# uncbiag/DeepAtlas

Measured on AMD Instinct MI355X. Metric: training volumes/sec at 160x192x160 fp32; Dice vs CPU ref, higher is better.
Workload: dtype f32; 1 GPU; seg-only UNet_light + softmax-Dice + Adam training step, batch 2/GPU, 160x192x160 fp32 (BASELINE configs[1]); global_batch=2, n_classes=32, parallelism=dp1, matrix_precision=fp32_split, hip_graph=False, matrix_arithmetic_bits=22

## Files before the change

deepatlas_amd/_native.py:

```python
import ctypes
import os
from ctypes import c_int, c_float, c_longlong, c_size_t, c_void_p, c_char_p, POINTER

import torch

_HERE = os.path.dirname(os.path.abspath(__file__))
LIB_PATH = os.environ.get('DA_LIB') or os.path.join(_HERE, 'csrc', 'libdeepatlas_hip.so')

P = c_void_p
I = c_int
F = c_float
LL = c_longlong
SZ = c_size_t

SIGNATURES = {
    'da_version': (I, []),
    'da_device_info': (I, [POINTER(c_int), POINTER(c_int), POINTER(c_size_t), c_char_p, I]),
    'da_w_oik_to_tio': (I, [P, P, I, I, I, P]),
    'da_w_tio_to_oik': (I, [P, P, I, I, I, P]),
    'da_w_iok_to_tio': (I, [P, P, I, I, I, P]),
    'da_w_tio_to_iok': (I, [P, P, I, I, I, P]),
    'da_w_iok_flip_to_tio': (I, [P, P, I, I, I, P]),
    'da_w_tio_to_iok_flip': (I, [P, P, I, I, I, P]),
    'da_w_tio_to_oik_acc': (I, [P, P, I, I, I, P]),
    'da_w_tio_to_iok_acc': (I, [P, P, I, I, I, P]),
    'da_w_tio_to_iok_flip_acc': (I, [P, P, I, I, I, P]),
    'da_conv3d_k3_ws_bytes': (SZ, [I, I, I, I, I, I, I]),
    'da_conv3d_k3_pack_bytes': (SZ, [I, I, I, I, I, I]),
    'da_conv3d_k3_dgrad_bst': (I, [P, P, P, I, P, I, I, I, I, I, I, P, P, F, P, I, P, P, SZ, P]),
    'da_conv3d_k3_prepack': (I, [P, I, I, I, I, I, I, I, I, P, SZ, P, SZ, P, P]),
    'da_conv3d_k3_use_prepacked': (None, [P, P, SZ, P, SZ]),
    'da_conv3d_k3_prepack_many': (I, [I, P, P, P, P, P, P, P, P, P, P, P, P, P, P, P]),
    'da_conv3d_k3_fwd': (I, [P, I, P, I, P, P, P, I, I, I, I, I, I, F, P, SZ, P]),
    'da_conv3d_k3_fwd_bnstats': (I, [P, I, P, I, P, P, P, I, I, I, I, I, I, P, I, POINTER(c_int), P, SZ, P]),
    'da_conv3d_k3_dgrad': (I, [P, P, P, I, P, I, I, I, I, I, I, I, P, SZ, P]),
    'da_conv3d_k3_wgrad': (I, [P, I, P, I, P, P, P, I, I, I, I, I, I, P, SZ, P]),
    'da_conv3d_k3_fwd_pro': (I, [P, I, P, P, F, P, I, P, P, F, P, P, P, I, I, I, I, I, F, P, I, POINTER(c_int), P, SZ, P]),
    'da_conv3d_k3_wgrad_pro': (I, [P, I, P, P, F, P, I, P, P, F, P, P, I, I, I, I, I, P, SZ, P]),
    'da_upconv3d_k3_supported': (I, [I, I, I]),
    'da_upconv3d_k3_ws_bytes': (SZ, [I, I, I, I, I, I]),
    'da_upconv3d_k3_fwd': (I, [P, I, P, I, P, P, P, I, I, I, I, I, F, P, SZ, P]),
    'da_upconv3d_k3_dgrad': (I, [P, P, P, I, P, I, I, I, I, I, I, P, SZ, P]),
    'da_upconv3d_k3_wgrad': (I, [P, I, P, I, P, P, I, I, I, I, I, P, SZ, P]),
    'da_set_conv_direct': (I, [I]),
    'da_set_matrix_bf16': (I, [I]),
    'da_set_matrix_mode': (I, [I]),
    'da_pointwise_ws_bytes': (SZ, [I, I, I]),
    'da_conv1x1_fwd': (I, [P, P, P, P, LL, I, I, P, SZ, P]),
    'da_conv1x1_fwd_pro': (I, [P, P, P, F, P, P, P, LL, I, I, P, SZ, P]),
    'da_conv1x1_wgrad_pro': (I, [P, P, P, F, P, P, P, LL, I, I, P, SZ, P]),
    'da_conv1x1_dgrad': (I, [P, P, P, LL, I, I, P, SZ, P]),
    'da_conv1x1_wgrad_ws_bytes': (SZ, [LL, I, I]),
    'da_conv1x1_wgrad': (I, [P, P, P, P, LL, I, I, P, SZ, P]),
    'da_deconv_k2s2_fwd': (I, [P, P, P, P, I, I, I, I, I, I, P, SZ, P]),
    'da_deconv_k2s2_fwd_bnstats': (I, [P, P, P, P, I, I, I, I, I, I, P, I, POINTER(c_int), P, SZ, P]),
    'da_deconv_k2s2_dgrad': (I, [P, P, P, I, I, I, I, I, I, P, SZ, P]),
    'da_deconv_k2s2_bn_bwd_ws_bytes': (SZ, [I, I, I, I, I, I]),
    'da_deconv_k2s2_bn_bwd': (I, [P, P, P, P, P, P, F, P, P, P, P, P, P, P, I, I, I, I, I, I, P, I, P, SZ, P]),
    'da_deconv_k2s2_wgrad_ws_bytes': (SZ, [I, I, I, I, I, I]),
    'da_deconv_k2s2_wgrad': (I, [P, P, P, P, I, I, I, I, I, I, P, SZ, P]),
    'da_bn_ws_bytes': (SZ, [LL, I]),
    'da_bn_train_stats': (I, [P, LL, I, P, P, F, F, P, P, P, P, P, P, P, SZ, P]),
    'da_bn_train_stats_from_partials': (I, [P, I, LL, I, P, P, F, F, P, P, P, P, P, P, P]),
    'da_bn_eval_affine': (I, [P, P, P, P, F, I, P, P, P, P, P]),
    'da_bn_act_fwd': (I, [P, P, P, F, P, LL, I, P]),
    'da_bn_act_bwd': (I, [P, P, P, P, P, P, P, F, I, P, P, P, LL, I, P, SZ, P]),
    'da_bn_act_bwd_dbias': (I, [P, P, P, P, P, P, F, I, P, P, P, P, LL, I, P, SZ, P]),
    'da_bn_act_bwd_dbias_pre': (I, [P, P, P, P, P, P, F, I, P, P, P, P, LL, I, P, I, P, SZ, P]),
    'da_act_bwd': (I, [P, P, F, P, LL, P]),
    'da_act_bwd_add_dbias': (I, [P, P, P, F, P, P, LL, I, P, SZ, P]),
    'da_colsum': (I, [P, LL, I, P, P, SZ, P]),
    'da_act_bwd_add_partial': (I, [P, P, P, F, P, LL, I, P, SZ, POINTER(c_int), P]),
    'da_colsum_finish': (I, [P, I, I, P, I, P]),
    'da_maxpool2_fwd': (I, [P, P, I, I, I, I, I, P]),
    'da_maxpool2_fwd_pro': (I, [P, P, P, F, P, P, I, I, I, I, I, P]),
    'da_maxpool2_bwd': (I, [P, P, P, I, I, I, I, I, P]),
    'da_maxpool2_bwd_add': (I, [P, P, P, P, I, I, I, I, I, P]),
    'da_maxpool2_bwd_bst': (I, [P, P, P, P, I, I, I, I, I, P, F, P, I, P, P]),
    'da_upsample_nearest_fwd': (I, [P, P, I, I, I, I, I, I, I, I, P]),
    'da_upsample_nearest_bwd': (I, [P, P, I, I, I, I, I, I, I, I, P]),
    'da_warp_fwd': (I, [P, P, P, P, I, I, I, I, I, P]),
    'da_warp_bwd': (I, [P, P, P, P, P, I, I, I, I, I, P]),
    'da_label_warp_dice_ws_bytes': (SZ, [I, I]),
    'da_warp_dice_ws_bytes': (SZ, [I, I]),
    'da_warp_dice_fwd': (I, [P, P, P, I, I, I, I, I, I, I, I, F, P, P, P, SZ, P]),
    'da_softmax_dice_fwd': (I, [P, P, I, P, I, LL, I, I, I, F, P, P, P, SZ, P]),
    'da_label_warp_dice_fwd': (I, [P, I, P, I, P, I, I, I, I, I, I, I, F, P, P, P, SZ, P]),
    'da_label_warp_dice_bwd': (I, [P, I, P, I, P, P, P, P, I, I, I, I, I, P]),
    'da_softwarp_dice_ws_bytes': (SZ, [I, I]),
    'da_softwarp_dice_fwd': (I, [P, I, P, P, I, I, I, I, I, I, I, I, F, P, P, P, SZ, P]),
    'da_softwarp_dice_bwd_disp': (I, [P, I, P, P, P, P, P, I, I, I, I, I, P]),
    'da_softwarp_dice_bwd_logits': (I, [P, I, P, P, P, P, P, I, I, I, I, I, P]),
    'da_warp_adjoint_labels': (I, [P, I, P, P, P, I, I, I, I, I, P]),
    'da_seg_anat_dlogits': (I, [P, P, I, P, P, P, P, P, P, P, I, LL, I, P]),
    'da_warp_bwd_dsrc_det_ws_bytes': (SZ, [I, I, I, I, I]),
    'da_warp_bwd_dsrc_det': (I, [P, P, P, I, I, I, I, I, P, SZ, P]),
    'da_identity_grid': (I, [P, I, I, I, I, P]),
    'da_warp_labels_fwd': (I, [P, I, P, P, I, I, I, I, I, P]),
    'da_warp_labels_bwd': (I, [P, P, I, P, P, I, I, I, I, I, P]),
    'da_dice_ws_bytes': (SZ, [I, LL, I]),
    'da_dice_fwd': (I, [P, P, I, P, I, LL, I, I, I, I, F, P, P, P, SZ, P]),
    'da_dice_bwd': (I, [P, P, I, P, P, P, P, I, LL, I, I, P]),
    'da_softmax_fwd': (I, [P, P, LL, I, P]),
    'da_softmax_bwd': (I, [P, P, P, LL, I, P]),
    'da_one_hot': (I, [P, I, P, LL, I, P]),
    'da_head_dice_ws_bytes': (SZ, [I, LL, I, I]),
    'da_head_dice_fwd': (I, [P, P, P, F, P, P, P, I, I, LL, I, I, I, I, F, P, P, P, SZ, P]),
    'da_head_dice_bwd': (I, [P, P, P, F, P, P, P, I, P, P, P, P, P, I, LL, I, I, P, SZ, P]),
    'da_head_dice_bwd_bst': (I, [P, P, P, F, P, P, P, P, I, P, P, P, P, P, I, LL, I, I, P, I, P, P, SZ, P]),
    'da_ncc_ws_bytes': (SZ, [I, LL]),
    'da_ncc_fwd': (I, [P, P, I, LL, P, P, P, SZ, P]),
    'da_ncc_bwd': (I, [P, P, P, P, P, P, I, LL, P]),
    'da_bending_ws_bytes': (SZ, [I, I, I, I]),
    'da_bending_fwd': (I, [P, I, I, I, I, P, I, I, P, P, SZ, P]),
    'da_bending_bwd': (I, [P, P, P, I, I, I, I, P, I, I, P]),
    'da_xent_ws_bytes': (SZ, []),
    'da_xent_fwd': (I, [P, P, I, P, P, LL, I, I, I, F, LL, I, P, P, P, SZ, P]),
    'da_xent_bwd': (I, [P, P, I, P, P, P, P, P, LL, I, I, I, F, LL, P]),
    'da_argmax_dice_counts': (I, [P, P, I, I, LL, I, P, P, P]),
    'da_label_overlap_counts': (I, [P, I, P, I, I, LL, I, P, P]),
    'da_warp_labels_nearest_counts': (I, [P, I, P, I, P, I, I, I, I, I, P, P, P]),
    'da_jacobian_det_ws_bytes': (SZ, [I, I, I, I]),
    'da_jacobian_det': (I, [P, I, I, I, I, P, P, P, SZ, P]),
    'da_jacdet_penalty_ws_bytes': (SZ, [I, I, I, I]),
    'da_jacdet_penalty_fwd': (I, [P, I, I, I, I, F, I, P, P, P, P, SZ, P]),
    'da_jacdet_penalty_bwd': (I, [P, P, P, P, I, I, I, I, F, I, P]),
    'da_invcons_ws_bytes': (SZ, [I, I, I, I]),
    'da_invcons_fwd': (I, [P, P, I, I, I, I, P, P, P, P, SZ, P]),
    'da_invcons_bwd': (I, [P, P, P, P, P, P, I, I, I, I, I, P, SZ, P]),
    'da_field_invert_ws_bytes': (SZ, [I, I, I, I]),
    'da_field_invert': (I, [P, P, P, I, I, I, I, I, F, P, P, SZ, P]),
    'da_field_points_ws_bytes': (SZ, [I, I]),
    'da_field_transport_points': (I, [P, P, P, I, I, I, I, I, I, I, F, P, P, SZ, P]),
    'da_affine_warp_fwd': (I, [P, P, P, I, I, I, I, I, P]),
    'da_affine_warp_ws_bytes': (SZ, [I, I, I, I]),
    'da_affine_warp_bwd_theta': (I, [P, P, P, P, I, I, I, I, I, P, SZ, P]),
    'da_affine_compose_disp': (I, [P, P, P, I, I, I, I, P]),
    'da_label_fusion_vote': (I, [P, I, LL, P, P, P, I, I, I, I, I, P, P, P]),
    'da_local_msd_weights_ws_bytes': (SZ, [I, I, I, I, I]),
    'da_local_msd_weights': (I, [P, P, I, I, I, I, I, I, F, P, P, SZ, P]),
    'da_conv_k2s2_fwd': (I, [P, P, P, P, I, I, I, I, I, I, P, SZ, P]),
    'da_conv_k2s2_dgrad': (I, [P, P, P, I, I, I, I, I, I, P, SZ, P]),
    'da_conv_k2s2_wgrad_ws_bytes': (SZ, [I, I, I, I, I, I]),
    'da_conv_k2s2_wgrad': (I, [P, P, P, P, I, I, I, I, I, I, P, SZ, P]),
    'da_upsample_trilinear2_fwd': (I, [P, P, I, I, I, I, I, P]),
    'da_upsample_trilinear2_bwd': (I, [P, P, I, I, I, I, I, P]),
    'da_clamp01_to_f32': (I, [P, I, P, LL, P]),
    'da_crop3d': (I, [P, P, I, LL, I, I, I, I, I, I, I, I, I, P]),
    'da_partition_tiles': (I, [P, P, I, I, I, I, P, P, P]),
    'da_assemble_tiles': (I, [P, P, I, I, I, I, P, P, I, P]),
    'da_synth_volume': (I, [P, P, I, I, I, I, I, I, F, ctypes.c_uint, I, P]),
    'da_spatial_resample': (I, [P, P, I, I, P, P, I, P, P, I, I, I, I, I, I, I, I, P]),
    'da_lncc_ws_bytes': (SZ, [I, I, I, I, I, I, I]),
    'da_lncc_fwd': (I, [P, P, I, I, I, I, I, I, I, F, P, P, P, SZ, P]),
    'da_lncc_bwd': (I, [P, P, P, P, P, P, I, I, I, I, I, I, I, F, P, SZ, P]),
    'da_mi_ws_bytes': (SZ, [I, LL, I]),
    'da_mi_fwd': (I, [P, P, I, LL, I, F, F, F, P, P, P, SZ, P]),
    'da_mi_bwd': (I, [P, P, P, P, P, P, I, LL, I, F, F, F, P]),
    'da_gradloss_ws_bytes': (SZ, [I, I, I, I]),
    'da_gradloss_fwd': (I, [P, I, I, I, I, P, I, I, P, P, SZ, P]),
    'da_gradloss_bwd': (I, [P, P, P, I, I, I, I, P, I, I, P]),
    'da_adam_step': (I, [P, P, P, P, LL, F, F, F, F, I, F, P]),
    'da_adam_host_state': (I, [F, F, F, F, I, F, P]),
    'da_adam_step_dev': (I, [P, P, P, P, LL, P, P]),
}

BF16_TWINS = ['da_bn_train_stats', 'da_bn_act_fwd', 'da_bn_act_bwd_dbias', 'da_act_bwd', 'da_act_bwd_add_dbias', 'da_act_bwd_add_partial', 'da_colsum',
              'da_maxpool2_fwd', 'da_maxpool2_fwd_pro', 'da_maxpool2_bwd', 'da_maxpool2_bwd_add', 'da_upsample_nearest_fwd', 'da_upsample_nearest_bwd',
              'da_deconv_k2s2_fwd', 'da_deconv_k2s2_fwd_bnstats', 'da_deconv_k2s2_dgrad', 'da_deconv_k2s2_wgrad',
              'da_conv1x1_fwd', 'da_conv1x1_fwd_pro', 'da_conv1x1_dgrad', 'da_conv1x1_wgrad', 'da_conv1x1_wgrad_pro', 'da_head_dice_fwd', 'da_head_dice_bwd']
BF16_MASKED_TWINS = ['da_conv3d_k3_fwd', 'da_conv3d_k3_fwd_bnstats', 'da_conv3d_k3_fwd_pro', 'da_conv3d_k3_wgrad_pro', 'da_conv3d_k3_dgrad', 'da_conv3d_k3_wgrad']
for _n in BF16_TWINS:
    SIGNATURES[_n + '_bf16'] = (SIGNATURES[_n][0], list(SIGNATURES[_n][1]))
for _n in BF16_MASKED_TWINS:
    SIGNATURES[_n + '_bf16'] = (SIGNATURES[_n][0], list(SIGNATURES[_n][1]) + [ctypes.c_uint])
SIGNATURES['da_cast_f32_to_bf16'] = (I, [P, P, LL, P])
SIGNATURES['da_cast_bf16_to_f32'] = (I, [P, P, LL, P])

_lib = None


class NativeError(RuntimeError):
    pass


def lib():
    global _lib
    if _lib is None:
        if not os.path.isfile(LIB_PATH):
            raise NativeError(
                "deepatlas_amd: %s is missing. Build it with `python -c 'import __graft_entry__ as g; g.build()'` "
                "(hipcc --offload-arch=gfx950). There is no CPU/eager fallback for the hot path." % LIB_PATH)
        l = ctypes.CDLL(LIB_PATH)
        for name, (res, args) in SIGNATURES.items():
            fn = getattr(l, name)
            fn.restype = res
            fn.argtypes = args
        _lib = l
    return _lib


_ERR = {-1: 'DA_ERR_BADARG', -2: 'DA_ERR_WS_SMALL', -3: 'DA_ERR_UNSUPPORTED'}


class CallProfiler:

    def __init__(self, names=None):
        self.names = set(names) if names else None
        self.records = {}

    def wants(self, name):
        return self.names is None or name in self.names

    def summary(self):
        out = {}
        for key, evs in self.records.items():
            out[key] = (len(evs), sum(a.elapsed_time(b) for a, b in evs))
        return out


profiler = None
n_calls = 0


def call(name, *args):
    global n_calls
    n_calls += 1
    prof = profiler
    base = name[:-5] if name.endswith('_bf16') else name
    if prof is not None and prof.wants(base):
        a, b = torch.cuda.Event(enable_timing=True), torch.cuda.Event(enable_timing=True)
        a.record()
        rc = getattr(lib(), name)(*args)
        b.record()
        key = (base, tuple(x for x in args if isinstance(x, int)) + (('bf16',) if base != name else ()))
        prof.records.setdefault(key, []).append((a, b))
    else:
        rc = getattr(lib(), name)(*args)
    if rc != 0:
        raise NativeError('%s failed: %s' % (name, _ERR.get(rc, 'hipError_t %d' % rc)))


def call_supported(name, *args):
    try:
        call(name, *args)
        return True
    except NativeError as e:
        if 'DA_ERR_UNSUPPORTED' in str(e):
            return False
        raise


def ptr(t):
    if t is None:
        return None
    return c_void_p(t.data_ptr())


def stream():
    return c_void_p(torch.cuda.current_stream().cuda_stream)


def require_cuda(*tensors):
    for t in tensors:
        if t is not None and not t.is_cuda:
            raise NativeError("deepatlas_amd ops run only on the GPU (HIP kernels); got a CPU tensor. "
                              "The CPU restatement lives in oracle/ and is test infrastructure only.")


class _Workspace:

    def __init__(self):
        self.buf = {}
        self.capture_tag = None

    def get(self, nbytes, device):
        nbytes = int(nbytes) + 256
        key = (device.type, device.index if device.index is not None else torch.cuda.current_device(), torch.cuda.current_stream().cuda_stream)
        if self.capture_tag is not None and torch.cuda.is_current_stream_capturing():
            key = key + (self.capture_tag, len([k for k in self.buf if k[:3] == key and len(k) == 5 and k[3] == self.capture_tag]))
            for k, b in self.buf.items():
                if len(k) == 5 and k[:4] == key[:4] and b.numel() >= nbytes:
                    return c_void_p(b.data_ptr()), c_size_t(b.numel())
        b = self.buf.get(key)
        if b is None or b.numel() < nbytes:
            b = torch.empty(int(nbytes * 1.25) + 4096, dtype=torch.uint8, device=device)
            self.buf[key] = b
        return c_void_p(b.data_ptr()), c_size_t(b.numel())


    def release(self, tag):
        for k in [k for k in self.buf if len(k) == 5 and k[3] == tag]:
            del self.buf[k]


workspace = _Workspace()
```

deepatlas_amd/csrc/headdice.hip:

```cpp
#include "common.h"

typedef float f32x4 __attribute__((ext_vector_type(4)));

namespace {

constexpr int kHdBlocks = 1024;
constexpr int MT = 4;
constexpr float kLog2e = 1.44269504088896341f;

struct HdP {
    const float* x; const float* ps; const float* pt; float pslope;
    const float* wp_fwd; const float* wp_bwd; const float* bias;
    const void* labels; int label_bytes;
    long long V; int N, K, C;
    double* partial;
    const float* coef; const float* dloss;
    float* dx; float* wpartial;
    const float* pmean; double* bst;
};

__device__ __forceinline__ float hd_act01(float z, float s) { return fmaxf(z, z * s); }
__device__ __forceinline__ long long hd_label(const void* labels, int label_bytes, long long i) {
    return label_bytes == 1 ? (long long)((const unsigned char*)labels)[i] : ((const long long*)labels)[i];
}

__global__ void hd_pack_kernel(const float* __restrict__ w, float* __restrict__ wp, int K, int N, int transposed) {
    const int KC = K / 16, NT = N / 16;
    const int total = NT * KC * 256;
    for (int idx = blockIdx.x * blockDim.x + threadIdx.x; idx < total; idx += gridDim.x * blockDim.x) {
        const int m = idx & 3, lane = (idx >> 2) & 63;
        int rest = idx >> 8;
        const int c = rest % KC; const int n = rest / KC;
        const int k = 16 * c + 4 * (lane >> 4) + m, j = 16 * n + (lane & 15);
        wp[idx] = transposed ? w[(size_t)j * K + k] : w[(size_t)k * N + j];
    }
}

typedef float f2 __attribute__((ext_vector_type(2)));
__device__ __forceinline__ f2 hd_lo(f32x4 v) { return __builtin_shufflevector(v, v, 0, 1); }
__device__ __forceinline__ f2 hd_hi(f32x4 v) { return __builtin_shufflevector(v, v, 2, 3); }
__device__ __forceinline__ f2 hd_bc(float x) { return (f2){x, x}; }

template <int KC, typename T>
__device__ __forceinline__ void hd_load(const HdP& p, const T* __restrict__ xs, long long vbase, int i, int g, float4 (&a)[MT][KC]) {
#pragma unroll
    for (int t = 0; t < MT; ++t) {
        const long long vox = min(vbase + t * 16 + i, p.V - 1);
#pragma unroll
        for (int c = 0; c < KC; ++c) a[t][c] = da_ldq(xs, (vox * p.K + 16 * c + 4 * g) >> 2);
    }
}
__device__ __forceinline__ void hd_labels(const HdP& p, long long lbase, long long vbase, int i, int g, int (&rel)[MT]) {
#pragma unroll
    for (int t = 0; t < MT; ++t) rel[t] = (int)((const unsigned char*)p.labels)[(lbase + min(vbase + t * 16 + i, p.V - 1)) * p.label_bytes];
}
__device__ __forceinline__ int hd_rel(const HdP& p, int lab, long long vox, int g) { return (vox < p.V ? lab : -1000) - 4 * g; }
template <int NT>
__device__ __forceinline__ void hd_mask(int rel, f2 (&mk)[NT][2]) {
#pragma unroll
    for (int n = 0; n < NT; ++n) {
        mk[n][0] = (f2){rel == 16 * n ? 1.f : 0.f, rel == 16 * n + 1 ? 1.f : 0.f};
        mk[n][1] = (f2){rel == 16 * n + 2 ? 1.f : 0.f, rel == 16 * n + 3 ? 1.f : 0.f};
    }
}

template <int KC, int NT, typename T = float>
__device__ __forceinline__ void hd_probs(const HdP& p, long long vbase, int i, int g, const float4 (&psc)[KC], const float4 (&psf)[KC],
                                         const float4 (&wf)[NT][KC], const float (&bv)[NT][4], float4 (&a)[MT][KC], f32x4 (&acc)[MT][NT]) {
    if (p.ps) {
#pragma unroll
        for (int c = 0; c < KC; ++c) {
            const float4 sc = psc[c], sf = psf[c];
#pragma unroll
            for (int t = 0; t < MT; ++t) {
                a[t][c].x = hd_act01(a[t][c].x * sc.x + sf.x, p.pslope); a[t][c].y = hd_act01(a[t][c].y * sc.y + sf.y, p.pslope);
                a[t][c].z = hd_act01(a[t][c].z * sc.z + sf.z, p.pslope); a[t][c].w = hd_act01(a[t][c].w * sc.w + sf.w, p.pslope);
                if constexpr (DaEl<T>::bf) a[t][c] = da_unpack_bf16x4(da_pack_bf16x4(a[t][c]));
            }
        }
    }
#pragma unroll
    for (int t = 0; t < MT; ++t)
#pragma unroll
        for (int n = 0; n < NT; ++n) acc[t][n] = (f32x4){bv[n][0], bv[n][1], bv[n][2], bv[n][3]};
#pragma unroll
    for (int c = 0; c < KC; ++c) {
#pragma unroll
        for (int n = 0; n < NT; ++n)
#pragma unroll
            for (int t = 0; t < MT; ++t) acc[t][n] = __builtin_amdgcn_mfma_f32_16x16x4f32(wf[n][c].x, a[t][c].x, acc[t][n], 0, 0, 0);
#pragma unroll
        for (int n = 0; n < NT; ++n)
#pragma unroll
            for (int t = 0; t < MT; ++t) acc[t][n] = __builtin_amdgcn_mfma_f32_16x16x4f32(wf[n][c].y, a[t][c].y, acc[t][n], 0, 0, 0);
#pragma unroll
        for (int n = 0; n < NT; ++n)
#pragma unroll
            for (int t = 0; t < MT; ++t) acc[t][n] = __builtin_amdgcn_mfma_f32_16x16x4f32(wf[n][c].z, a[t][c].z, acc[t][n], 0, 0, 0);
#pragma unroll
        for (int n = 0; n < NT; ++n)
#pragma unroll
            for (int t = 0; t < MT; ++t) acc[t][n] = __builtin_amdgcn_mfma_f32_16x16x4f32(wf[n][c].w, a[t][c].w, acc[t][n], 0, 0, 0);
    }
#pragma unroll
    for (int t = 0; t < MT; ++t) {
        const bool valid = vbase + t * 16 + i < p.V;
        float m = acc[t][0][0];
#pragma unroll
        for (int n = 0; n < NT; ++n)
#pragma unroll
            for (int reg = 0; reg < 4; ++reg) m = fmaxf(m, acc[t][n][reg]);
        m = da_rows_max(m);
        f2 s2 = (f2){0.f, 0.f};
#pragma unroll
        for (int n = 0; n < NT; ++n) {
#pragma unroll
            for (int reg = 0; reg < 4; ++reg) acc[t][n][reg] = __builtin_amdgcn_exp2f(acc[t][n][reg] - m);
            s2 += hd_lo(acc[t][n]) + hd_hi(acc[t][n]);
        }
        const float s = da_rows_sum(s2.x + s2.y);
        const f2 inv = hd_bc(valid ? __builtin_amdgcn_rcpf(s) : 0.f);
#pragma unroll
        for (int n = 0; n < NT; ++n) {
            const f2 lo = hd_lo(acc[t][n]) * inv, hi = hd_hi(acc[t][n]) * inv;
            acc[t][n] = (f32x4){lo.x, lo.y, hi.x, hi.y};
        }
    }
}

template <int NT>
__device__ __forceinline__ void hd_bias(const HdP& p, int g, float (&bv)[NT][4]) {
#pragma unroll
    for (int n = 0; n < NT; ++n)
#pragma unroll
        for (int reg = 0; reg < 4; ++reg) bv[n][reg] = p.bias ? p.bias[16 * n + 4 * g + reg] * kLog2e : 0.f;
}
template <int KC, int NT>
__device__ __forceinline__ void hd_weights(const HdP& p, int lane, float4 (&wf)[NT][KC]) {
#pragma unroll
    for (int n = 0; n < NT; ++n)
#pragma unroll
        for (int c = 0; c < KC; ++c) {
            const float4 w = reinterpret_cast<const float4*>(p.wp_fwd)[(n * KC + c) * 64 + lane];
            wf[n][c] = make_float4(w.x * kLog2e, w.y * kLog2e, w.z * kLog2e, w.w * kLog2e);
        }
}
template <int KC>
__device__ __forceinline__ void hd_prologue(const HdP& p, int g, float4 (&psc)[KC], float4 (&psf)[KC]) {
#pragma unroll
    for (int c = 0; c < KC; ++c) {
        psc[c] = p.ps ? *reinterpret_cast<const float4*>(p.ps + 16 * c + 4 * g) : make_float4(1.f, 1.f, 1.f, 1.f);
        psf[c] = p.ps ? *reinterpret_cast<const float4*>(p.pt + 16 * c + 4 * g) : make_float4(0.f, 0.f, 0.f, 0.f);
    }
}

template <int KC, int NT, typename T = float>
__global__ void __launch_bounds__(256) head_dice_fwd_kernel(HdP p) {
    __shared__ double sred[4][3][NT * 16];
    const int lane = threadIdx.x & 63, wave = threadIdx.x >> 6;
    const int i = lane & 15, g = lane >> 4;
    const int n_s = blockIdx.y;
    const T* xs = reinterpret_cast<const T*>(p.x) + (long long)n_s * p.V * p.K;
    const long long lbase = (long long)n_s * p.V;
    float4 wf[NT][KC]; float bv[NT][4]; float4 psc[KC], psf[KC];
    hd_bias<NT>(p, g, bv);
    hd_weights<KC, NT>(p, lane, wf);
    hd_prologue<KC>(p, g, psc, psf);
    f2 sI[NT][2], sS[NT][2], sT[NT][2];
#pragma unroll
    for (int n = 0; n < NT; ++n)
#pragma unroll
        for (int h = 0; h < 2; ++h) sI[n][h] = sS[n][h] = sT[n][h] = (f2){0.f, 0.f};
    const long long nchunks = (p.V + 255) / 256;
    float4 an[MT][KC]; int reln[MT];
    if ((long long)blockIdx.x < nchunks) { hd_load<KC, T>(p, xs, (long long)blockIdx.x * 256 + wave * 64, i, g, an); hd_labels(p, lbase, (long long)blockIdx.x * 256 + wave * 64, i, g, reln); }
    for (long long cb = blockIdx.x; cb < nchunks; cb += gridDim.x) {
        const long long vbase = cb * 256 + wave * 64;
        float4 a[MT][KC]; f32x4 acc[MT][NT]; int rel[MT];
#pragma unroll
        for (int t = 0; t < MT; ++t) {
            rel[t] = hd_rel(p, reln[t], vbase + t * 16 + i, g);
#pragma unroll
            for (int c = 0; c < KC; ++c) a[t][c] = an[t][c];
        }
        { const long long vn = min(cb + (long long)gridDim.x, nchunks - 1) * 256 + wave * 64; hd_load<KC, T>(p, xs, vn, i, g, an); hd_labels(p, lbase, vn, i, g, reln); }
        hd_probs<KC, NT, T>(p, vbase, i, g, psc, psf, wf, bv, a, acc);
#pragma unroll
        for (int t = 0; t < MT; ++t) {
            f2 mk[NT][2];
            hd_mask<NT>(rel[t], mk);
#pragma unroll
            for (int n = 0; n < NT; ++n) {
                const f2 lo = hd_lo(acc[t][n]), hi = hd_hi(acc[t][n]);
                sS[n][0] += lo; sS[n][1] += hi;
                sI[n][0] += lo * mk[n][0]; sI[n][1] += hi * mk[n][1];
                sT[n][0] += mk[n][0]; sT[n][1] += mk[n][1];
            }
        }
    }
#pragma unroll
    for (int n = 0; n < NT; ++n)
#pragma unroll
        for (int reg = 0; reg < 4; ++reg) {
            double a0 = (double)sI[n][reg >> 1][reg & 1], a1 = (double)sS[n][reg >> 1][reg & 1], a2 = (double)sT[n][reg >> 1][reg & 1];
#pragma unroll
            for (int o = 1; o < 16; o <<= 1) { a0 += __shfl_xor(a0, o); a1 += __shfl_xor(a1, o); a2 += __shfl_xor(a2, o); }
            if (i == 0) { const int c = 16 * n + 4 * g + reg; sred[wave][0][c] = a0; sred[wave][1][c] = a1; sred[wave][2][c] = a2; }
        }
    __syncthreads();
    for (int idx = threadIdx.x; idx < 3 * p.C; idx += blockDim.x) {
        const int k = idx / p.C, c = idx % p.C;
        p.partial[(((size_t)n_s * gridDim.x + blockIdx.x) * 3 + k) * p.C + c] = (sred[0][k][c] + sred[1][k][c]) + (sred[2][k][c] + sred[3][k][c]);
    }
}

template <int KC, int NT, typename T = float>
__global__ void __launch_bounds__(256) head_dice_bwd_kernel(HdP p) {
    constexpr int K = KC * 16, C = NT * 16, LDX = K + 4, LDD = C + 4;
    extern __shared__ __attribute__((aligned(16))) float lds[];
    const int lane = threadIdx.x & 63, wave = threadIdx.x >> 6;
    const int i = lane & 15, g = lane >> 4;
    float* xl = lds + wave * (64 * LDX + 64 * LDD);
    float* dl = xl + 64 * LDX;
    float4 wf[NT][KC]; float bv[NT][4]; float4 psc[KC], psf[KC];
    hd_bias<NT>(p, g, bv);
    hd_weights<KC, NT>(p, lane, wf);
    hd_prologue<KC>(p, g, psc, psf);
    float wd[KC][NT][4];
#pragma unroll
    for (int c = 0; c < KC; ++c)
#pragma unroll
        for (int n = 0; n < NT; ++n)
#pragma unroll
            for (int reg = 0; reg < 4; ++reg) wd[c][n][reg] = p.wp_bwd[(size_t)(16 * c + i) * C + 16 * n + 4 * g + reg];
    const float gl = p.dloss[0];
    f32x4 wacc[KC][NT];
#pragma unroll
    for (int c = 0; c < KC; ++c)
#pragma unroll
        for (int n = 0; n < NT; ++n) wacc[c][n] = (f32x4){0.f, 0.f, 0.f, 0.f};
    f2 db[NT][2];
#pragma unroll
    for (int n = 0; n < NT; ++n) db[n][0] = db[n][1] = (f2){0.f, 0.f};
    const bool bst = KC == 1 && p.bst != nullptr;
    float4 bsc = make_float4(0.f, 0.f, 0.f, 0.f), bsf = bsc, bmu = bsc;
    float bs1[4] = {0.f, 0.f, 0.f, 0.f}, bs2[4] = {0.f, 0.f, 0.f, 0.f};
    if (bst) { bsc = *reinterpret_cast<const float4*>(p.ps + 4 * g); bsf = *reinterpret_cast<const float4*>(p.pt + 4 * g); bmu = *reinterpret_cast<const float4*>(p.pmean + 4 * g); }
    const long long chunks_per_sample = (p.V + 255) / 256, nchunks = chunks_per_sample * p.N;
    float4 an[MT][KC]; int reln[MT];
    auto fetch = [&](long long cb) {
        const int n_s = (int)(cb / chunks_per_sample);
        const long long vbase = (cb - (long long)n_s * chunks_per_sample) * 256 + wave * 64;
        hd_load<KC, T>(p, reinterpret_cast<const T*>(p.x) + (long long)n_s * p.V * p.K, vbase, i, g, an);
        hd_labels(p, (long long)n_s * p.V, vbase, i, g, reln);
    };
    if ((long long)blockIdx.x < nchunks) fetch(blockIdx.x);
    for (long long cb = blockIdx.x; cb < nchunks; cb += gridDim.x) {
        const int n_s = (int)(cb / chunks_per_sample);
        const long long vbase = (cb - (long long)n_s * chunks_per_sample) * 256 + wave * 64;
        const T* xs = reinterpret_cast<const T*>(p.x) + (long long)n_s * p.V * p.K;
        T* dxs = reinterpret_cast<T*>(p.dx) + (long long)n_s * p.V * p.K;
        const float* c0 = p.coef + (size_t)n_s * p.C;
        const float* c1 = p.coef + (size_t)(p.N + n_s) * p.C;
        float4 a[MT][KC]; f32x4 acc[MT][NT]; int rel[MT];
#pragma unroll
        for (int t = 0; t < MT; ++t) {
            rel[t] = hd_rel(p, reln[t], vbase + t * 16 + i, g);
#pragma unroll
            for (int c = 0; c < KC; ++c) a[t][c] = an[t][c];
        }
        fetch(min(cb + (long long)gridDim.x, nchunks - 1));
        hd_probs<KC, NT, T>(p, vbase, i, g, psc, psf, wf, bv, a, acc);
#pragma unroll
        for (int t = 0; t < MT; ++t)
#pragma unroll
            for (int c = 0; c < KC; ++c) *reinterpret_cast<float4*>(xl + (t * 16 + i) * LDX + 16 * c + 4 * g) = a[t][c];
        f2 k0[NT][2], k1[NT][2];
#pragma unroll
        for (int n = 0; n < NT; ++n)
#pragma unroll
            for (int h = 0; h < 2; ++h) {
                k0[n][h] = (f2){c0[16 * n + 4 * g + 2 * h], c0[16 * n + 4 * g + 2 * h + 1]};
                k1[n][h] = (f2){c1[16 * n + 4 * g + 2 * h], c1[16 * n + 4 * g + 2 * h + 1]};
            }
#pragma unroll
        for (int t = 0; t < MT; ++t) {
            f2 mk[NT][2], gg[NT][2], pr[NT][2], dot2 = (f2){0.f, 0.f};
            hd_mask<NT>(rel[t], mk);
#pragma unroll
            for (int n = 0; n < NT; ++n) {
                pr[n][0] = hd_lo(acc[t][n]); pr[n][1] = hd_hi(acc[t][n]);
#pragma unroll
                for (int h = 0; h < 2; ++h) { gg[n][h] = k0[n][h] * mk[n][h] + k1[n][h]; dot2 += gg[n][h] * pr[n][h]; }
            }
            const f2 dot = hd_bc(da_rows_sum(dot2.x + dot2.y)), gl2 = hd_bc(gl);
#pragma unroll
            for (int n = 0; n < NT; ++n) {
                const f2 d0 = (gl2 * pr[n][0]) * (gg[n][0] - dot), d1 = (gl2 * pr[n][1]) * (gg[n][1] - dot);
                db[n][0] += d0; db[n][1] += d1;
                acc[t][n] = (f32x4){d0.x, d0.y, d1.x, d1.y};
                *reinterpret_cast<float4*>(dl + (t * 16 + i) * LDD + 16 * n + 4 * g) = make_float4(d0.x, d0.y, d1.x, d1.y);
            }
        }
#pragma unroll
        for (int t = 0; t < MT; ++t) {
            f32x4 dacc[KC];
#pragma unroll
            for (int c = 0; c < KC; ++c) dacc[c] = (f32x4){0.f, 0.f, 0.f, 0.f};
#pragma unroll
            for (int n = 0; n < NT; ++n)
#pragma unroll
                for (int reg = 0; reg < 4; ++reg)
#pragma unroll
                    for (int c = 0; c < KC; ++c) dacc[c] = __builtin_amdgcn_mfma_f32_16x16x4f32(wd[c][n][reg], acc[t][n][reg], dacc[c], 0, 0, 0);
            const long long vox = vbase + t * 16 + i;
            if (vox < p.V) {
#pragma unroll
                for (int c = 0; c < KC; ++c)
                    da_stq_nt(dxs, (vox * p.K + 16 * c + 4 * g) >> 2, make_float4(dacc[c][0], dacc[c][1], dacc[c][2], dacc[c][3]));
                if (bst) {
                    const float4 xr = da_ldq(xs, (vox * p.K + 4 * g) >> 2);
                    const float xv[4] = {xr.x, xr.y, xr.z, xr.w}, scv[4] = {bsc.x, bsc.y, bsc.z, bsc.w}, sfv[4] = {bsf.x, bsf.y, bsf.z, bsf.w}, muv[4] = {bmu.x, bmu.y, bmu.z, bmu.w};
#pragma unroll
                    for (int j = 0; j < 4; ++j) {
                        const float dz = dacc[0][j] * da_act_grad(xv[j] * scv[j] + sfv[j], p.pslope >= 1.f ? -1.f : p.pslope);
                        bs1[j] += dz; bs2[j] += dz * (xv[j] - muv[j]);
                    }
                }
            }
        }
        __builtin_amdgcn_wave_barrier();
#pragma unroll 4
        for (int s = 0; s < 16; ++s) {
            float av[KC], bw[NT];
#pragma unroll
            for (int c = 0; c < KC; ++c) av[c] = xl[(4 * s + g) * LDX + 16 * c + i];
#pragma unroll
            for (int n = 0; n < NT; ++n) bw[n] = dl[(4 * s + g) * LDD + 16 * n + i];
#pragma unroll
            for (int c = 0; c < KC; ++c)
#pragma unroll
                for (int n = 0; n < NT; ++n) wacc[c][n] = __builtin_amdgcn_mfma_f32_16x16x4f32(av[c], bw[n], wacc[c][n], 0, 0, 0);
        }
        __builtin_amdgcn_wave_barrier();
    }
    __syncthreads();
    float* red = lds;
    for (int w = 0; w < 4; ++w) {
        if (wave == w) {
#pragma unroll
            for (int c = 0; c < KC; ++c)
#pragma unroll
                for (int n = 0; n < NT; ++n)
#pragma unroll
                    for (int reg = 0; reg < 4; ++reg) {
                        const int idx = (16 * c + 4 * g + reg) * C + 16 * n + i;
                        red[idx] = (w == 0 ? 0.f : red[idx]) + wacc[c][n][reg];
                    }
#pragma unroll
            for (int n = 0; n < NT; ++n)
#pragma unroll
                for (int reg = 0; reg < 4; ++reg) {
                    float d = db[n][reg >> 1][reg & 1];
#pragma unroll
                    for (int o = 1; o < 16; o <<= 1) d += __shfl_xor(d, o);
                    const int cidx = K * C + 16 * n + 4 * g + reg;
                    if (i == 0) red[cidx] = (w == 0 ? 0.f : red[cidx]) + d;
                }
        }
        __syncthreads();
    }
    float* part = p.wpartial + (size_t)blockIdx.x * (K * C + C);
    for (int idx = threadIdx.x; idx < K * C + C; idx += blockDim.x) part[idx] = red[idx];
    if (bst) {
        __syncthreads();
        double* dred = reinterpret_cast<double*>(lds);
#pragma unroll
        for (int j = 0; j < 4; ++j) {
            double a0 = (double)bs1[j], a1 = (double)bs2[j];
#pragma unroll
            for (int o = 1; o < 16; o <<= 1) { a0 += __shfl_xor(a0, o); a1 += __shfl_xor(a1, o); }
            if (i == 0) { dred[(wave * 2 + 0) * 16 + 4 * g + j] = a0; dred[(wave * 2 + 1) * 16 + 4 * g + j] = a1; }
        }
        __syncthreads();
        if (threadIdx.x < 32) {
            const int k = threadIdx.x >> 4, c = threadIdx.x & 15;
            p.bst[((size_t)blockIdx.x * 2 + k) * 16 + c] = (dred[(0 * 2 + k) * 16 + c] + dred[(1 * 2 + k) * 16 + c]) + (dred[(2 * 2 + k) * 16 + c] + dred[(3 * 2 + k) * 16 + c]);
        }
    }
}

static bool hd_shape_ok(int K, int C) { return (K == 16 || K == 64) && (C == 16 || C == 32); }

}

extern "C" size_t da_head_dice_ws_bytes(int N, long long V, int Cin, int C) {
    (void)V;
    const size_t pack = da_align((size_t)2 * Cin * C * sizeof(float));
    const size_t fwd = da_align((size_t)N * kHdBlocks * 3 * C * sizeof(double)) + da_align((size_t)3 * N * C * sizeof(float));
    const size_t bwd = da_align((size_t)kHdBlocks * (Cin * C + C) * sizeof(float)) + da_align((size_t)(Cin * C + C) * sizeof(float));
    return pack + (fwd > bwd ? fwd : bwd);
}

template <int KC, int NT, typename T>
static int hd_launch_fwd(const HdP& p, int nblocks, hipStream_t st) {
    hipLaunchKernelGGL((head_dice_fwd_kernel<KC, NT, T>), dim3(nblocks, p.N), dim3(256), 0, st, p);
    DA_LAUNCH_CHECK();
    return 0;
}
template <int KC, int NT, typename T>
static int hd_launch_bwd(const HdP& p, int nblocks, hipStream_t st) {
    const size_t shm = (size_t)4 * (64 * (KC * 16 + 4) + 64 * (NT * 16 + 4)) * sizeof(float);
    return da_launch_lds<head_dice_bwd_kernel<KC, NT, T>>(dim3(nblocks), dim3(256), shm, st, p);
}

template <typename T>
static int head_dice_fwd_t(const float* x, const float* pro_scale, const float* pro_shift, float pro_slope,
                           const float* w_io, const float* bias, const void* labels, int label_bytes,
                           int N, long long V, int Cin, int C, int weight_type, int no_bg, float eps,
                           float* loss, float* coef, void* ws, size_t ws_bytes, void* stream) {
    if (!x || !w_io || !labels || !loss || !coef || N <= 0 || N > 64 || V <= 0 || (label_bytes != 1 && label_bytes != 8) ||
        ((pro_scale == nullptr) != (pro_shift == nullptr))) return DA_ERR_BADARG;
    if (!hd_shape_ok(Cin, C) || (pro_scale && pro_slope >= 1.f)) return DA_ERR_UNSUPPORTED;
    if (ws_bytes < da_head_dice_ws_bytes(N, V, Cin, C)) return DA_ERR_WS_SMALL;
    hipStream_t st = da_stream(stream);
    float* wp = (float*)ws;
    hipLaunchKernelGGL(hd_pack_kernel, dim3(da_grid(Cin * C, 256, 64)), dim3(256), 0, st, w_io, wp, Cin, C, 0);
    DA_LAUNCH_CHECK();
    char* rest = (char*)ws + da_align((size_t)2 * Cin * C * sizeof(float));
    double* partial = (double*)rest;
    float* isc = (float*)(rest + da_align((size_t)N * kHdBlocks * 3 * C * sizeof(double)));
    int nblocks = (int)da_cdiv(V, 256 * 2); if (nblocks > kHdBlocks) nblocks = kHdBlocks; if (nblocks < 1) nblocks = 1;
    HdP p;
    p.x = x; p.ps = pro_scale; p.pt = pro_shift; p.pslope = pro_scale ? (pro_slope < 0.f ? 1.f : pro_slope) : 1.f;
    p.wp_fwd = wp; p.wp_bwd = nullptr; p.bias = bias; p.labels = labels; p.label_bytes = label_bytes;
    p.V = V; p.N = N; p.K = Cin; p.C = C; p.partial = partial; p.coef = nullptr; p.dloss = nullptr; p.dx = nullptr; p.wpartial = nullptr; p.pmean = nullptr; p.bst = nullptr;
    int rc;
    if (Cin == 16 && C == 32) rc = hd_launch_fwd<1, 2, T>(p, nblocks, st);
    else if (Cin == 16 && C == 16) rc = hd_launch_fwd<1, 1, T>(p, nblocks, st);
    else if (Cin == 64 && C == 32) rc = hd_launch_fwd<4, 2, T>(p, nblocks, st);
    else rc = hd_launch_fwd<4, 1, T>(p, nblocks, st);
    if (rc) return rc;
    return da_dice_finish(partial, nblocks, N, C, weight_type, no_bg, eps, loss, coef, isc, st);
}
extern "C" int da_head_dice_fwd(const float* x, const float* pro_scale, const float* pro_shift, float pro_slope,
                                const float* w_io, const float* bias, const void* labels, int label_bytes,
                                int N, long long V, int Cin, int C, int weight_type, int no_bg, float eps,
                                float* loss, float* coef, void* ws, size_t ws_bytes, void* stream) {
    return head_dice_fwd_t<float>(x, pro_scale, pro_shift, pro_slope, w_io, bias, labels, label_bytes, N, V, Cin, C, weight_type, no_bg, eps, loss, coef, ws, ws_bytes, stream);
}
extern "C" int da_head_dice_fwd_bf16(const void* x, const float* pro_scale, const float* pro_shift, float pro_slope,
                                     const float* w_io, const float* bias, const void* labels, int label_bytes,
                                     int N, long long V, int Cin, int C, int weight_type, int no_bg, float eps,
                                     float* loss, float* coef, void* ws, size_t ws_bytes, void* stream) {
    return head_dice_fwd_t<da_bf16>((const float*)x, pro_scale, pro_shift, pro_slope, w_io, bias, labels, label_bytes, N, V, Cin, C, weight_type, no_bg, eps, loss, coef, ws, ws_bytes, stream);
}

template <typename T>
static int head_dice_bwd_t(const float* x, const float* pro_scale, const float* pro_shift, float pro_slope,
                           const float* w_io, const float* bias, const void* labels, int label_bytes,
                           const float* coef, const float* dloss, float* dx, float* dw_io, float* dbias,
                           int N, long long V, int Cin, int C, void* ws, size_t ws_bytes, void* stream,
                           const float* pro_mean = nullptr, double* bst = nullptr, int bst_cap = 0, int* bst_n = nullptr) {
    if (bst_n) *bst_n = 0;
    if (!x || !w_io || !labels || !coef || !dloss || !dx || !dw_io || N <= 0 || V <= 0 || (label_bytes != 1 && label_bytes != 8) ||
        ((pro_scale == nullptr) != (pro_shift == nullptr))) return DA_ERR_BADARG;
    if (!hd_shape_ok(Cin, C) || (pro_scale && pro_slope >= 1.f)) return DA_ERR_UNSUPPORTED;
    if (ws_bytes < da_head_dice_ws_bytes(N, V, Cin, C)) return DA_ERR_WS_SMALL;
    hipStream_t st = da_stream(stream);
    float* wpf = (float*)ws;
    const float* wpb = w_io;
    hipLaunchKernelGGL(hd_pack_kernel, dim3(da_grid(Cin * C, 256, 64)), dim3(256), 0, st, w_io, wpf, Cin, C, 0);
    DA_LAUNCH_CHECK();
    char* rest = (char*)ws + da_align((size_t)2 * Cin * C * sizeof(float));
    float* wpartial = (float*)rest;
    const int O = Cin * C + C;
    float* folded = (float*)(rest + da_align((size_t)kHdBlocks * O * sizeof(float)));
    const long long nchunks = da_cdiv(V, 256) * N;
    int nblocks = (int)(nchunks < kHdBlocks ? nchunks : kHdBlocks); if (nblocks < 1) nblocks = 1;
    HdP p;
    p.x = x; p.ps = pro_scale; p.pt = pro_shift; p.pslope = pro_scale ? (pro_slope < 0.f ? 1.f : pro_slope) : 1.f;
    p.wp_fwd = wpf; p.wp_bwd = wpb; p.bias = bias; p.labels = labels; p.label_bytes = label_bytes;
    p.V = V; p.N = N; p.K = Cin; p.C = C; p.partial = nullptr; p.coef = coef; p.dloss = dloss; p.dx = dx; p.wpartial = wpartial;
    const bool want_bst = bst && pro_scale && pro_mean && Cin == 16 && bst_cap >= nblocks && !DaEl<T>::bf;
    p.pmean = want_bst ? pro_mean : nullptr; p.bst = want_bst ? bst : nullptr;
    if (want_bst && bst_n) *bst_n = nblocks;
    int rc;
    if (Cin == 16 && C == 32) rc = hd_launch_bwd<1, 2, T>(p, nblocks, st);
    else if (Cin == 16 && C == 16) rc = hd_launch_bwd<1, 1, T>(p, nblocks, st);
    else if (Cin == 64 && C == 32) rc = hd_launch_bwd<4, 2, T>(p, nblocks, st);
    else rc = hd_launch_bwd<4, 1, T>(p, nblocks, st);
    if (rc) return rc;
    rc = da_reduce_partials(wpartial, nblocks, O, folded, st);
    if (rc) return rc;
    hipError_t e = hipMemcpyAsync(dw_io, folded, (size_t)Cin * C * sizeof(float), hipMemcpyDeviceToDevice, st);
    if (e != hipSuccess) return (int)e;
    if (dbias) { e = hipMemcpyAsync(dbias, folded + (size_t)Cin * C, (size_t)C * sizeof(float), hipMemcpyDeviceToDevice, st); if (e != hipSuccess) return (int)e; }
    return 0;
}
extern "C" int da_head_dice_bwd(const float* x, const float* pro_scale, const float* pro_shift, float pro_slope,
                                const float* w_io, const float* bias, const void* labels, int label_bytes,
                                const float* coef, const float* dloss, float* dx, float* dw_io, float* dbias,
                                int N, long long V, int Cin, int C, void* ws, size_t ws_bytes, void* stream) {
    return head_dice_bwd_t<float>(x, pro_scale, pro_shift, pro_slope, w_io, bias, labels, label_bytes, coef, dloss, dx, dw_io, dbias, N, V, Cin, C, ws, ws_bytes, stream);
}
extern "C" int da_head_dice_bwd_bst(const float* x, const float* pro_scale, const float* pro_shift, float pro_slope, const float* pro_mean,
                                    const float* w_io, const float* bias, const void* labels, int label_bytes,
                                    const float* coef, const float* dloss, float* dx, float* dw_io, float* dbias,
                                    int N, long long V, int Cin, int C, double* bst, int bst_cap, int* bst_n, void* ws, size_t ws_bytes, void* stream) {
    return head_dice_bwd_t<float>(x, pro_scale, pro_shift, pro_slope, w_io, bias, labels, label_bytes, coef, dloss, dx, dw_io, dbias, N, V, Cin, C, ws, ws_bytes, stream,
                                  pro_mean, bst, bst_cap, bst_n);
}
extern "C" int da_head_dice_bwd_bf16(const void* x, const float* pro_scale, const float* pro_shift, float pro_slope,
                                     const float* w_io, const float* bias, const void* labels, int label_bytes,
                                     const float* coef, const float* dloss, void* dx, float* dw_io, float* dbias,
                                     int N, long long V, int Cin, int C, void* ws, size_t ws_bytes, void* stream) {
    return head_dice_bwd_t<da_bf16>((const float*)x, pro_scale, pro_shift, pro_slope, w_io, bias, labels, label_bytes, coef, dloss, (float*)dx, dw_io, dbias, N, V, Cin, C, ws, ws_bytes, stream);
}
```

deepatlas_amd/csrc/losses.hip:

```cpp
#include "common.h"

namespace {

constexpr int kBlocks = 512;
constexpr int kBendBlocks = 4096;
constexpr int kDiceBlocks = 2048;

__device__ __forceinline__ long long load_label(const void* labels, int label_bytes, long long i) {
    return label_bytes == 1 ? (long long)((const unsigned char*)labels)[i] : ((const long long*)labels)[i];
}

__device__ __forceinline__ void group_softmax4(float (&x)[4], int lpv) {
    float m = fmaxf(fmaxf(x[0], x[1]), fmaxf(x[2], x[3]));
    for (int o = 1; o < lpv; o <<= 1) m = fmaxf(m, __shfl_xor(m, o));
    float s = 0.f;
#pragma unroll
    for (int j = 0; j < 4; ++j) { x[j] = expf(x[j] - m); s += x[j]; }
    for (int o = 1; o < lpv; o <<= 1) s += __shfl_xor(s, o);
    const float inv = 1.f / s;
#pragma unroll
    for (int j = 0; j < 4; ++j) x[j] *= inv;
}

__global__ void dice_partial_vec_kernel(const float* __restrict__ src, const void* __restrict__ labels, int label_bytes,
                                        const float* __restrict__ soft, long long V, int C, int lpv, int softmax,
                                        double* __restrict__ partial, float* __restrict__ prob_out = nullptr) {
    extern __shared__ float shf[];
    const int n = blockIdx.y;
    const int slots = blockDim.x / lpv;
    const int q = threadIdx.x % lpv, s = threadIdx.x / lpv;
    float aI[4] = {0, 0, 0, 0}, aS[4] = {0, 0, 0, 0}, aT[4] = {0, 0, 0, 0};
    const long long vpb = da_cdiv(V, (long long)gridDim.x);
    const long long v0 = (long long)blockIdx.x * vpb;
    long long v1 = v0 + vpb; if (v1 > V) v1 = V;
    auto accumulate = [&](float4 a, const float* tt, long long row) {
        float p[4] = {a.x, a.y, a.z, a.w};
        if (softmax) group_softmax4(p, lpv);
        if (prob_out) *reinterpret_cast<float4*>(prob_out + row * C + q * 4) = make_float4(p[0], p[1], p[2], p[3]);
#pragma unroll
        for (int j = 0; j < 4; ++j) { aI[j] += p[j] * tt[j]; aS[j] += p[j]; aT[j] += tt[j]; }
    };
    auto target = [&](long long row, float* tt) {
        if (soft) {
            const float4 b = *reinterpret_cast<const float4*>(soft + row * C + q * 4);
            tt[0] = b.x; tt[1] = b.y; tt[2] = b.z; tt[3] = b.w;
        } else {
            const int lab = (int)load_label(labels, label_bytes, row) - q * 4;
#pragma unroll
            for (int j = 0; j < 4; ++j) tt[j] = (lab == j) ? 1.f : 0.f;
        }
    };
    long long v = v0 + s;
    for (; v + slots < v1; v += 2 * slots) {
        const long long r0 = (long long)n * V + v, r1 = r0 + slots;
        const float4 a0 = *reinterpret_cast<const float4*>(src + r0 * C + q * 4);
        const float4 a1 = *reinterpret_cast<const float4*>(src + r1 * C + q * 4);
        float t0[4], t1[4];
        target(r0, t0); target(r1, t1);
        accumulate(a0, t0, r0); accumulate(a1, t1, r1);
    }
    for (; v < v1; v += slots) {
        const long long r0 = (long long)n * V + v;
        const float4 a0 = *reinterpret_cast<const float4*>(src + r0 * C + q * 4);
        float t0[4];
        target(r0, t0);
        accumulate(a0, t0, r0);
    }
    float* sI = shf; float* sS = shf + (size_t)slots * C; float* sT = shf + (size_t)2 * slots * C;
#pragma unroll
    for (int j = 0; j < 4; ++j) { sI[s * C + q * 4 + j] = aI[j]; sS[s * C + q * 4 + j] = aS[j]; sT[s * C + q * 4 + j] = aT[j]; }
    __syncthreads();
    for (int c = threadIdx.x; c < C; c += blockDim.x) {
        double tI = 0, tS = 0, tT = 0;
        for (int k = 0; k < slots; ++k) { tI += sI[k * C + c]; tS += sS[k * C + c]; tT += sT[k * C + c]; }
        double* o = partial + (((size_t)n * gridDim.x + blockIdx.x) * 3) * C;
        o[c] = tI; o[C + c] = tS; o[2 * C + c] = tT;
    }
}

__global__ void dice_partial_gen_kernel(const float* __restrict__ src, const void* __restrict__ labels, int label_bytes,
                                        const float* __restrict__ soft, long long V, int C, int softmax,
                                        double* __restrict__ partial) {
    extern __shared__ float shf[];
    const int n = blockIdx.y;
    for (int c = threadIdx.x; c < 4 * 3 * C; c += blockDim.x) shf[c] = 0.f;
    __syncthreads();
    float* mine = shf + (threadIdx.x >> 6) * 3 * C;
    const long long vpb = da_cdiv(V, (long long)gridDim.x);
    const long long v0 = (long long)blockIdx.x * vpb;
    long long v1 = v0 + vpb; if (v1 > V) v1 = V;
    const long long span = da_cdiv(v1 - v0, (long long)blockDim.x) * blockDim.x;
    for (long long k = threadIdx.x; k < span; k += blockDim.x) {
        const long long v = v0 + k;
        const bool live = v < v1;
        const long long row = (long long)n * V + (live ? v : v0);
        float m = -INFINITY, ssum = 1.f;
        if (softmax) {
            for (int c = 0; c < C; ++c) m = fmaxf(m, src[row * C + c]);
            ssum = 0.f;
            for (int c = 0; c < C; ++c) ssum += expf(src[row * C + c] - m);
        }
        const int lab = soft ? -1 : (int)load_label(labels, label_bytes, row);
        for (int c = 0; c < C; ++c) {
            float p = src[row * C + c];
            if (softmax) p = expf(p - m) / ssum;
            float t = soft ? soft[row * C + c] : (lab == c ? 1.f : 0.f);
            if (!live) { p = 0.f; t = 0.f; }
            const float wI = da_wave_sum(p * t), wS = da_wave_sum(p), wT = da_wave_sum(t);
            if ((threadIdx.x & 63) == 0) { mine[c] += wI; mine[C + c] += wS; mine[2 * C + c] += wT; }
        }
    }
    __syncthreads();
    for (int c = threadIdx.x; c < C; c += blockDim.x) {
        double* o = partial + (((size_t)n * gridDim.x + blockIdx.x) * 3) * C;
        double a = 0.0, b = 0.0, t = 0.0;
        for (int w = 0; w < 4; ++w) { a += shf[w * 3 * C + c]; b += shf[w * 3 * C + C + c]; t += shf[w * 3 * C + 2 * C + c]; }
        o[c] = a; o[C + c] = b; o[2 * C + c] = t;
    }
}

__global__ void colreduce_inplace_kernel(double* __restrict__ partial, int N, int nblocks, int R) {
    const int wave = (int)((blockIdx.x * blockDim.x + threadIdx.x) >> 6), lane = threadIdx.x & 63;
    if (wave >= N * R) return;
    const int n = wave / R, r = wave % R;
    double* col = partial + (size_t)n * nblocks * R + r;
    double s = 0.0;
    for (int b = lane; b < nblocks; b += 64) s += col[(size_t)b * R];
    s = da_wave_sum(s);
    if (lane == 0) col[0] = s;
}

__global__ void dice_finalize_kernel(const double* __restrict__ partial, int nblocks, int nsum, int N, int C,
                                     int weight_type, int no_bg, float eps, float* __restrict__ loss,
                                     float* __restrict__ coef, float* __restrict__ isc ) {
    const int NC = N * C;
    for (int i = threadIdx.x; i < 3 * NC; i += blockDim.x) {
        const int k = i / NC, nc = i % NC, n = nc / C, c = nc % C;
        double s = 0.0;
        for (int b = 0; b < nsum; ++b) s += partial[(((size_t)n * nblocks + b) * 3 + k) * C + c];
        isc[i] = (float)s;
    }
    __syncthreads();
    if (threadIdx.x != 0) return;
    const float* I = isc; const float* S = isc + NC; const float* T = isc + 2 * NC;
    const int c0 = no_bg ? 1 : 0;
    float wmax = -INFINITY;
    for (int n = 0; n < N; ++n) {
        float rowmax = -INFINITY;
        for (int c = c0; c < C; ++c) {
            float w;
            if (weight_type == 1) w = 1.f / (powf(T[n * C + c], (float)(1.0 / 3.0)) + eps);
            else if (weight_type == 2) w = 1.f / (T[n * C + c] + eps);
            else w = 1.f;
            coef[n * C + c] = w;
            if (weight_type == 2) { const float t = isinf(w) ? 1.f : w; rowmax = fmaxf(rowmax, t); }
        }
        for (int c = c0; c < C; ++c) {
            float w = coef[n * C + c];
            if (weight_type == 2 && isinf(w)) { w = rowmax; coef[n * C + c] = w; }
            wmax = fmaxf(wmax, w);
        }
    }
    float wsum = 0.f, acc = 0.f;
    for (int n = 0; n < N; ++n)
        for (int c = c0; c < C; ++c) {
            const float w = coef[n * C + c] / wmax;
            coef[n * C + c] = w;
            const float score = (2.f * I[n * C + c] + eps) / ((S[n * C + c] + T[n * C + c]) + 2.f * eps);
            acc += w * score; wsum += w;
        }
    loss[0] = 1.f - acc / wsum;
    for (int n = 0; n < N; ++n)
        for (int c = 0; c < C; ++c) {
            if (c < c0) { coef[n * C + c] = 0.f; coef[NC + n * C + c] = 0.f; continue; }
            const float w = coef[n * C + c] / wsum;
            const float den = (S[n * C + c] + T[n * C + c]) + 2.f * eps;
            coef[n * C + c] = -w * 2.f / den;
            coef[NC + n * C + c] = w * (2.f * I[n * C + c] + eps) / (den * den);
        }
}

__global__ void dice_bwd_vec_kernel(const float* __restrict__ src, const void* __restrict__ labels, int label_bytes,
                                    const float* __restrict__ soft, const float* __restrict__ coef,
                                    const float* __restrict__ dloss, float* __restrict__ d_src,
                                    int N, long long V, int C, int lpv, int softmax) {
    const long long total = (long long)N * V * lpv;
    const float gl = dloss[0];
    const int NC = N * C;
    for (long long i = (long long)blockIdx.x * blockDim.x + threadIdx.x; i < total; i += (long long)gridDim.x * blockDim.x) {
        const int q = (int)(i % lpv);
        const long long row = i / lpv;
        const int n = (int)(row / V);
        const float4 a = *reinterpret_cast<const float4*>(src + row * C + q * 4);
        float p[4] = {a.x, a.y, a.z, a.w};
        if (softmax) group_softmax4(p, lpv);
        float t[4];
        if (soft) {
            const float4 b = *reinterpret_cast<const float4*>(soft + row * C + q * 4);
            t[0] = b.x; t[1] = b.y; t[2] = b.z; t[3] = b.w;
        } else {
            const int lab = (int)load_label(labels, label_bytes, row) - q * 4;
#pragma unroll
            for (int j = 0; j < 4; ++j) t[j] = (lab == j) ? 1.f : 0.f;
        }
        float g[4];
#pragma unroll
        for (int j = 0; j < 4; ++j) g[j] = coef[n * C + q * 4 + j] * t[j] + coef[NC + n * C + q * 4 + j];
        float4 o;
        if (softmax) {
            float dot = g[0] * p[0] + g[1] * p[1] + g[2] * p[2] + g[3] * p[3];
            for (int k = 1; k < lpv; k <<= 1) dot += __shfl_xor(dot, k);
            o = make_float4(gl * p[0] * (g[0] - dot), gl * p[1] * (g[1] - dot), gl * p[2] * (g[2] - dot), gl * p[3] * (g[3] - dot));
        } else {
            o = make_float4(gl * g[0], gl * g[1], gl * g[2], gl * g[3]);
        }
        *reinterpret_cast<float4*>(d_src + row * C + q * 4) = o;
    }
}

__global__ void dice_bwd_gen_kernel(const float* __restrict__ src, const void* __restrict__ labels, int label_bytes,
                                    const float* __restrict__ soft, const float* __restrict__ coef,
                                    const float* __restrict__ dloss, float* __restrict__ d_src,
                                    int N, long long V, int C, int softmax) {
    const long long total = (long long)N * V;
    const float gl = dloss[0];
    const int NC = N * C;
    for (long long row = (long long)blockIdx.x * blockDim.x + threadIdx.x; row < total; row += (long long)gridDim.x * blockDim.x) {
        const int n = (int)(row / V);
        const int lab = soft ? -1 : (int)load_label(labels, label_bytes, row);
        float m = -INFINITY, ssum = 1.f, dot = 0.f;
        if (softmax) {
            for (int c = 0; c < C; ++c) m = fmaxf(m, src[row * C + c]);
            ssum = 0.f;
            for (int c = 0; c < C; ++c) ssum += expf(src[row * C + c] - m);
            for (int c = 0; c < C; ++c) {
                const float p = expf(src[row * C + c] - m) / ssum;
                const float t = soft ? soft[row * C + c] : (lab == c ? 1.f : 0.f);
                dot += (coef[n * C + c] * t + coef[NC + n * C + c]) * p;
            }
        }
        for (int c = 0; c < C; ++c) {
            const float t = soft ? soft[row * C + c] : (lab == c ? 1.f : 0.f);
            const float g = coef[n * C + c] * t + coef[NC + n * C + c];
            if (softmax) { const float p = expf(src[row * C + c] - m) / ssum; d_src[row * C + c] = gl * p * (g - dot); }
            else d_src[row * C + c] = gl * g;
        }
    }
}

__global__ void softmax_fwd_kernel(const float* __restrict__ x, float* __restrict__ y, long long M, int C, int lpv) {
    if (lpv > 0) {
        const long long total = M * lpv;
        for (long long i = (long long)blockIdx.x * blockDim.x + threadIdx.x; i < total; i += (long long)gridDim.x * blockDim.x) {
            const int q = (int)(i % lpv); const long long row = i / lpv;
            const float4 a = *reinterpret_cast<const float4*>(x + row * C + q * 4);
            float p[4] = {a.x, a.y, a.z, a.w};
            group_softmax4(p, lpv);
            *reinterpret_cast<float4*>(y + row * C + q * 4) = make_float4(p[0], p[1], p[2], p[3]);
        }
    } else {
        for (long long row = (long long)blockIdx.x * blockDim.x + threadIdx.x; row < M; row += (long long)gridDim.x * blockDim.x) {
            float m = -INFINITY, s = 0.f;
            for (int c = 0; c < C; ++c) m = fmaxf(m, x[row * C + c]);
            for (int c = 0; c < C; ++c) s += expf(x[row * C + c] - m);
            for (int c = 0; c < C; ++c) y[row * C + c] = expf(x[row * C + c] - m) / s;
        }
    }
}

__global__ void softmax_bwd_kernel(const float* __restrict__ dy, const float* __restrict__ y, float* __restrict__ dx,
                                   long long M, int C, int lpv) {
    if (lpv > 0) {
        const long long total = M * lpv;
        for (long long i = (long long)blockIdx.x * blockDim.x + threadIdx.x; i < total; i += (long long)gridDim.x * blockDim.x) {
            const int q = (int)(i % lpv); const long long row = i / lpv;
            const float4 g = *reinterpret_cast<const float4*>(dy + row * C + q * 4);
            const float4 p = *reinterpret_cast<const float4*>(y + row * C + q * 4);
            float dot = g.x * p.x + g.y * p.y + g.z * p.z + g.w * p.w;
            for (int k = 1; k < lpv; k <<= 1) dot += __shfl_xor(dot, k);
            *reinterpret_cast<float4*>(dx + row * C + q * 4) = make_float4(p.x * (g.x - dot), p.y * (g.y - dot), p.z * (g.z - dot), p.w * (g.w - dot));
        }
    } else {
        for (long long row = (long long)blockIdx.x * blockDim.x + threadIdx.x; row < M; row += (long long)gridDim.x * blockDim.x) {
            float dot = 0.f;
            for (int c = 0; c < C; ++c) dot += dy[row * C + c] * y[row * C + c];
            for (int c = 0; c < C; ++c) dx[row * C + c] = y[row * C + c] * (dy[row * C + c] - dot);
        }
    }
}

__global__ void one_hot_kernel(const void* __restrict__ labels, int label_bytes, float* __restrict__ out, long long M, int C) {
    const long long total = M * C;
    for (long long i = (long long)blockIdx.x * blockDim.x + threadIdx.x; i < total; i += (long long)gridDim.x * blockDim.x) {
        const long long row = i / C; const int c = (int)(i % C);
        out[i] = ((int)load_label(labels, label_bytes, row) == c) ? 1.f : 0.f;
    }
}

static int lpv_for(int C) {
    if (C % 4 != 0) return 0;
    const int q = C / 4;
    if (q > 64 || (q & (q - 1)) != 0) return 0;
    return q;
}

template <bool ALIGNED>
__global__ void ncc_partial_kernel(const float* __restrict__ x, const float* __restrict__ y, long long V,
                                   double* __restrict__ partial ) {
    __shared__ double red[5][4];
    const int n = blockIdx.y;
    const float* xs = x + (long long)n * V; const float* ys = y + (long long)n * V;
    const float px = xs[0], py = ys[0];
    float a[5] = {0, 0, 0, 0, 0};
    double acc[5] = {0, 0, 0, 0, 0};
    long long head = 0;
    if (!ALIGNED) {
        head = (long long)(((16 - ((size_t)xs & 15)) & 15) >> 2);
        if ((((size_t)xs ^ (size_t)ys) & 15) != 0 || head > V) head = V;
    }
    const long long V4 = (V - head) / 4;
    const float* xb = xs + head; const float* yb = ys + head;
    int cnt = 0;
    for (long long i = (long long)blockIdx.x * blockDim.x + threadIdx.x; i < V4; i += (long long)gridDim.x * blockDim.x) {
        float4 p = reinterpret_cast<const float4*>(xb)[i];
        float4 q = reinterpret_cast<const float4*>(yb)[i];
        p.x -= px; p.y -= px; p.z -= px; p.w -= px;
        q.x -= py; q.y -= py; q.z -= py; q.w -= py;
        a[0] += (p.x + p.y) + (p.z + p.w);
        a[1] += (q.x + q.y) + (q.z + q.w);
        a[2] += (p.x * q.x + p.y * q.y) + (p.z * q.z + p.w * q.w);
        a[3] += (p.x * p.x + p.y * p.y) + (p.z * p.z + p.w * p.w);
        a[4] += (q.x * q.x + q.y * q.y) + (q.z * q.z + q.w * q.w);
        if (++cnt == 16) {
#pragma unroll
            for (int k = 0; k < 5; ++k) { acc[k] += (double)a[k]; a[k] = 0.f; }
            cnt = 0;
        }
    }
    if (ALIGNED) {
        if (blockIdx.x == 0) for (long long i = V4 * 4 + threadIdx.x; i < V; i += blockDim.x) {
            const float p = xs[i] - px, q = ys[i] - py;
            a[0] += p; a[1] += q; a[2] += p * q; a[3] += p * p; a[4] += q * q;
        }
    } else {
        const long long nscalar = V - V4 * 4;
        cnt = 0;
        for (long long j = (long long)blockIdx.x * blockDim.x + threadIdx.x; j < nscalar; j += (long long)gridDim.x * blockDim.x) {
            const long long i = j < head ? j : j + V4 * 4;
            const float p = xs[i] - px, q = ys[i] - py;
            a[0] += p; a[1] += q; a[2] += p * q; a[3] += p * p; a[4] += q * q;
            if (++cnt == 64) {
#pragma unroll
                for (int k = 0; k < 5; ++k) { acc[k] += (double)a[k]; a[k] = 0.f; }
                cnt = 0;
            }
        }
    }
#pragma unroll
    for (int k = 0; k < 5; ++k) acc[k] += (double)a[k];
    const int lane = threadIdx.x & 63, wid = threadIdx.x >> 6;
#pragma unroll
    for (int k = 0; k < 5; ++k) { const double w = da_wave_sum(acc[k]); if (lane == 0) red[k][wid] = w; }
    __syncthreads();
    if (threadIdx.x < 5) {
        double s = 0.0;
        for (int w = 0; w < (int)(blockDim.x >> 6); ++w) s += red[threadIdx.x][w];
        partial[((size_t)n * gridDim.x + blockIdx.x) * 5 + threadIdx.x] = s;
    }
}

__global__ void ncc_finalize_kernel(const double* __restrict__ partial, int nblocks, int nsum, int N, long long V,
                                    const float* __restrict__ x, const float* __restrict__ y,
                                    float* __restrict__ loss, double* __restrict__ stats) {
    __shared__ double sncc[64];
    const int n = threadIdx.x;
    if (n < N) {
        double s[5] = {0, 0, 0, 0, 0};
        for (int b = 0; b < nsum; ++b)
            for (int k = 0; k < 5; ++k) s[k] += partial[((size_t)n * nblocks + b) * 5 + k];
        const double M = (double)V;
        const double mx = s[0] / M, my = s[1] / M;
        const double cov = s[2] / M - mx * my;
        double vx = s[3] / M - mx * mx, vy = s[4] / M - my * my;
        const double ncc = cov / (sqrt(vx) * sqrt(vy));
        double* o = stats + (size_t)n * 8;
        o[0] = mx + (double)x[(long long)n * V]; o[1] = my + (double)y[(long long)n * V]; o[2] = cov; o[3] = vx; o[4] = vy; o[5] = ncc; o[6] = M; o[7] = 0.0;
        sncc[n] = ncc;
    }
    __syncthreads();
    if (threadIdx.x == 0) {
        double t = 0.0;
        for (int i = 0; i < N; ++i) t += sncc[i];
        loss[0] = (float)(1.0 - t / (double)N);
    }
}

__global__ void ncc_bwd_kernel(const float* __restrict__ x, const float* __restrict__ y, const double* __restrict__ stats,
                               const float* __restrict__ dloss, float* __restrict__ dx, float* __restrict__ dy,
                               int N, long long V) {
    const int n = blockIdx.y;
    const double* s = stats + (size_t)n * 8;
    const float mx = (float)s[0], my = (float)s[1];
    const double sxy = sqrt(s[3]) * sqrt(s[4]);
    const double k = -(double)dloss[0] / ((double)N * s[6]);
    const float ax = (float)(k / sxy), bx = (float)(-k * s[5] / s[3]);
    const float ay = (float)(k / sxy), by = (float)(-k * s[5] / s[4]);
    const float* xs = x + (long long)n * V; const float* ys = y + (long long)n * V;
    for (long long i = (long long)blockIdx.x * blockDim.x + threadIdx.x; i < V; i += (long long)gridDim.x * blockDim.x) {
        const float xt = xs[i] - mx, yt = ys[i] - my;
        if (dx) dx[(long long)n * V + i] = ax * yt + bx * xt;
        if (dy) dy[(long long)n * V + i] = ay * xt + by * yt;
    }
}

struct BendK { float k[3][6]; };

static BendK bending_coeffs(int N, int D, int H, int W, const float* spacing3, int normalize, int norm) {
    float sp[3] = {1.f, 1.f, 1.f};
    if (spacing3) { sp[0] = spacing3[0]; sp[1] = spacing3[1]; sp[2] = spacing3[2]; }
    if (normalize) { const float m = fminf(sp[0], fminf(sp[1], sp[2])); sp[0] /= m; sp[1] /= m; sp[2] /= m; }
    float dims[3] = {(float)D, (float)H, (float)W};
    if (normalize) { const float m = fminf(dims[0], fminf(dims[1], dims[2])); dims[0] /= m; dims[1] /= m; dims[2] /= m; }
    const float den[6] = {sp[0] * sp[0], sp[1] * sp[1], sp[2] * sp[2], sp[0] * sp[1], sp[1] * sp[2], sp[2] * sp[0]};
    const double Mint = (double)(D - 2) * (H - 2) * (W - 2);
    BendK K;
    for (int c = 0; c < 3; ++c)
        for (int t = 0; t < 6; ++t) {
            const float w = norm == 2 ? dims[c] * sp[c] / den[t] : 1.f;
            const double mult = (t < 3 ? 1.0 : 2.0) / (9.0 * 3.0 * (double)N * Mint);
            K.k[c][t] = (float)((double)(w * w) * mult);
        }
    return K;
}

#define BU(dd, hh, ww) u[((((long long)(dd)) * H + (hh)) * W + (ww)) * 3 + c]

struct F3 { float x, y, z; };
__device__ __forceinline__ F3 ld3(const float* __restrict__ u, long long vox) {
    const float* p = u + vox * 3;
    return F3{p[0], p[1], p[2]};
}

template <bool L1>
__global__ void bending_partial_kernel(const float* __restrict__ disp, int D, int H, int W, BendK K,
                                       double* __restrict__ partial) {
    __shared__ double red[4];
    const int n = blockIdx.y;
    const float* u = disp + (long long)n * D * H * W * 3;
    const int Di = D - 2, Hi = H - 2, Wi = W - 2;
    const long long total = (long long)Di * Hi * Wi;
    const long long sH = W, sD = (long long)H * W;
    float acc = 0.f; double dacc = 0.0; int cnt = 0;
    for (DaXcdLoop L = da_xcd_loop(total); L.i < L.end; L.i += L.step) {
        const long long i = L.i;
        long long r = i;
        const int w = (int)(r % Wi) + 1; r /= Wi;
        const int h = (int)(r % Hi) + 1; const int d = (int)(r / Hi) + 1;
        const long long p = ((long long)d * H + h) * W + w;
        const F3 c0 = ld3(u, p);
        const F3 dp = ld3(u, p + sD), dm = ld3(u, p - sD), hp = ld3(u, p + sH), hm = ld3(u, p - sH), wp = ld3(u, p + 1), wm = ld3(u, p - 1);
        const F3 dhpp = ld3(u, p + sD + sH), dhmm = ld3(u, p - sD - sH), dhpm = ld3(u, p + sD - sH), dhmp = ld3(u, p - sD + sH);
        const F3 hwpp = ld3(u, p + sH + 1), hwmm = ld3(u, p - sH - 1), hwpm = ld3(u, p + sH - 1), hwmp = ld3(u, p - sH + 1);
        const F3 dwpp = ld3(u, p + sD + 1), dwmm = ld3(u, p - sD - 1), dwpm = ld3(u, p + sD - 1), dwmp = ld3(u, p - sD + 1);
#define BEND_CH(f, c)                                                                                   \
        {                                                                                               \
            const float t0 = dp.f + dm.f - 2.f * c0.f, t1 = hp.f + hm.f - 2.f * c0.f, t2 = wp.f + wm.f - 2.f * c0.f;   \
            const float t3 = dhpp.f + dhmm.f - dhpm.f - dhmp.f;                                         \
            const float t4 = hwpp.f + hwmm.f - hwpm.f - hwmp.f;                                         \
            const float t5 = dwpp.f + dwmm.f - dwpm.f - dwmp.f;                                         \
            if (L1) acc += K.k[c][0] * fabsf(t0) + K.k[c][1] * fabsf(t1) + K.k[c][2] * fabsf(t2) + K.k[c][3] * fabsf(t3) + K.k[c][4] * fabsf(t4) + K.k[c][5] * fabsf(t5); \
            else acc += K.k[c][0] * t0 * t0 + K.k[c][1] * t1 * t1 + K.k[c][2] * t2 * t2 + K.k[c][3] * t3 * t3 + K.k[c][4] * t4 * t4 + K.k[c][5] * t5 * t5; \
        }
        BEND_CH(x, 0) BEND_CH(y, 1) BEND_CH(z, 2)
#undef BEND_CH
        if (++cnt == 16) { dacc += (double)acc; acc = 0.f; cnt = 0; }
    }
    dacc += (double)acc;
    const double s = da_block_sum(dacc, red);
    if (threadIdx.x == 0) partial[(size_t)n * gridDim.x + blockIdx.x] = s;
}

__global__ void scalar_finalize_kernel(const double* __restrict__ partial, int count, float* __restrict__ loss) {
    __shared__ double red[4];
    double s = 0.0;
    for (int i = threadIdx.x; i < count; i += blockDim.x) s += partial[i];
    s = da_block_sum(s, red);
    if (threadIdx.x == 0) loss[0] = (float)s;
}

template <bool L1>
__device__ __forceinline__ float bend_grad_elem(const float* __restrict__ u, int d, int h, int w, int c, int D, int H, int W, const BendK& K) {
    auto interior = [&](int dd, int hh, int ww) { return dd >= 1 && dd < D - 1 && hh >= 1 && hh < H - 1 && ww >= 1 && ww < W - 1; };
    auto f = [](float t) { return L1 ? (t > 0.f ? 1.f : (t < 0.f ? -1.f : 0.f)) : t; };
    float g = 0.f;
    {
        float s0 = 0.f, s1 = 0.f, s2 = 0.f;
        if (interior(d, h, w)) {
            const float u0 = BU(d, h, w);
            s0 -= 2.f * f(BU(d + 1, h, w) + BU(d - 1, h, w) - 2.f * u0);
            s1 -= 2.f * f(BU(d, h + 1, w) + BU(d, h - 1, w) - 2.f * u0);
            s2 -= 2.f * f(BU(d, h, w + 1) + BU(d, h, w - 1) - 2.f * u0);
        }
#pragma unroll
        for (int sgn = -1; sgn <= 1; sgn += 2) {
            if (interior(d + sgn, h, w)) s0 += f(BU(d + 2 * sgn, h, w) + BU(d, h, w) - 2.f * BU(d + sgn, h, w));
            if (interior(d, h + sgn, w)) s1 += f(BU(d, h + 2 * sgn, w) + BU(d, h, w) - 2.f * BU(d, h + sgn, w));
            if (interior(d, h, w + sgn)) s2 += f(BU(d, h, w + 2 * sgn) + BU(d, h, w) - 2.f * BU(d, h, w + sgn));
        }
        g += K.k[c][0] * s0 + K.k[c][1] * s1 + K.k[c][2] * s2;
    }
    {
        float s3 = 0.f, s4 = 0.f, s5 = 0.f;
#pragma unroll
        for (int sa = -1; sa <= 1; sa += 2)
#pragma unroll
            for (int sb = -1; sb <= 1; sb += 2) {
                const float cf = (float)(sa * sb);
                { const int qd = d - sa, qh = h - sb;
                  if (interior(qd, qh, w)) s3 += cf * f(BU(qd + 1, qh + 1, w) + BU(qd - 1, qh - 1, w) - BU(qd + 1, qh - 1, w) - BU(qd - 1, qh + 1, w)); }
                { const int qh = h - sa, qw = w - sb;
                  if (interior(d, qh, qw)) s4 += cf * f(BU(d, qh + 1, qw + 1) + BU(d, qh - 1, qw - 1) - BU(d, qh + 1, qw - 1) - BU(d, qh - 1, qw + 1)); }
                { const int qd = d - sa, qw = w - sb;
                  if (interior(qd, h, qw)) s5 += cf * f(BU(qd + 1, h, qw + 1) + BU(qd - 1, h, qw - 1) - BU(qd + 1, h, qw - 1) - BU(qd - 1, h, qw + 1)); }
            }
        g += K.k[c][3] * s3 + K.k[c][4] * s4 + K.k[c][5] * s5;
    }
    return g;
}

template <bool L1>
__global__ void bending_bwd_kernel(const float* __restrict__ disp, const float* __restrict__ dloss,
                                   float* __restrict__ d_disp, int D, int H, int W, BendK K) {
    const int n = blockIdx.y;
    const float* u = disp + (long long)n * D * H * W * 3;
    float* du = d_disp + (long long)n * D * H * W * 3;
    const long long total = (long long)D * H * W * 3;
    const float gl = (L1 ? 1.f : 2.f) * dloss[0];
    const long long sW = 3, sH = (long long)W * 3, sD = (long long)H * W * 3;
    for (DaXcdLoop L = da_xcd_loop(total, 768); L.i < L.end; L.i += L.step) {
        const long long i = L.i;
        const int c = (int)(i % 3); long long r = i / 3;
        const int w = (int)(r % W); r /= W;
        const int h = (int)(r % H); const int d = (int)(r / H);
        float g;
        const bool deep = !L1 && d >= 2 && d < D - 2 && h >= 2 && h < H - 2 && w >= 2 && w < W - 2;
        if (deep) {
            const float* q = u + i;
            const float c0 = q[0];
            const float d2 = q[2 * sD] + q[-2 * sD], d1 = q[sD] + q[-sD];
            const float h2 = q[2 * sH] + q[-2 * sH], h1 = q[sH] + q[-sH];
            const float w2 = q[2 * sW] + q[-2 * sW], w1 = q[sW] + q[-sW];
            const float dh = q[2 * sD + 2 * sH] + q[2 * sD - 2 * sH] + q[-2 * sD + 2 * sH] + q[-2 * sD - 2 * sH];
            const float hw = q[2 * sH + 2 * sW] + q[2 * sH - 2 * sW] + q[-2 * sH + 2 * sW] + q[-2 * sH - 2 * sW];
            const float dw = q[2 * sD + 2 * sW] + q[2 * sD - 2 * sW] + q[-2 * sD + 2 * sW] + q[-2 * sD - 2 * sW];
            g = K.k[c][0] * (d2 - 4.f * d1 + 6.f * c0) + K.k[c][1] * (h2 - 4.f * h1 + 6.f * c0) + K.k[c][2] * (w2 - 4.f * w1 + 6.f * c0) +
                K.k[c][3] * (4.f * c0 - 2.f * (d2 + h2) + dh) + K.k[c][4] * (4.f * c0 - 2.f * (h2 + w2) + hw) + K.k[c][5] * (4.f * c0 - 2.f * (d2 + w2) + dw);
        } else {
            g = bend_grad_elem<L1>(u, d, h, w, c, D, H, W, K);
        }
        du[i] = gl * g;
    }
}
#undef BU

__global__ void argmax_counts_kernel(const float* __restrict__ logits, const void* __restrict__ truth, int label_bytes,
                                     long long V, int C, int lpv, unsigned long long* __restrict__ counts,
                                     unsigned char* __restrict__ pred) {
    extern __shared__ unsigned int shc[];
    const int n = blockIdx.y;
    for (int c = threadIdx.x; c < 3 * C; c += blockDim.x) shc[c] = 0u;
    __syncthreads();
    const int L = lpv > 0 ? lpv : 1;
    const long long total = V * L;
    for (long long i = (long long)blockIdx.x * blockDim.x + threadIdx.x; i < total; i += (long long)gridDim.x * blockDim.x) {
        const int q = (int)(i % L); const long long v = i / L;
        const long long row = (long long)n * V + v;
        float best; int bi;
        if (lpv > 0) {
            const float4 a = *reinterpret_cast<const float4*>(logits + row * C + q * 4);
            best = a.x; bi = q * 4;
            if (a.y > best) { best = a.y; bi = q * 4 + 1; }
            if (a.z > best) { best = a.z; bi = q * 4 + 2; }
            if (a.w > best) { best = a.w; bi = q * 4 + 3; }
            for (int o = 1; o < lpv; o <<= 1) {
                const float ob = __shfl_xor(best, o); const int oi = __shfl_xor(bi, o);
                if (ob > best || (ob == best && oi < bi)) { best = ob; bi = oi; }
            }
        } else {
            best = logits[row * C]; bi = 0;
            for (int c = 1; c < C; ++c) { const float a = logits[row * C + c]; if (a > best) { best = a; bi = c; } }
        }
        if (q == 0) {
            const int t = (int)load_label(truth, label_bytes, row);
            atomicAdd(&shc[bi], 1u);
            if (t >= 0 && t < C) atomicAdd(&shc[C + t], 1u);
            if (t == bi) atomicAdd(&shc[2 * C + bi], 1u);
            if (pred) pred[row] = (unsigned char)bi;
        }
    }
    __syncthreads();
    for (int c = threadIdx.x; c < 3 * C; c += blockDim.x) {
        const int k = c / C, cc = c % C;
        if (shc[c]) atomicAdd(&counts[((size_t)n * C + cc) * 3 + k], (unsigned long long)shc[c]);
    }
}


__global__ void label_overlap_counts_kernel(const void* __restrict__ pred, int pred_bytes, const void* __restrict__ truth, int truth_bytes,
                                            long long V, int C, unsigned long long* __restrict__ counts) {
    extern __shared__ unsigned int shc[];
    constexpr int RUN = 16;
    const int n = blockIdx.y;
    for (int c = threadIdx.x; c < 4 * 3 * C; c += blockDim.x) shc[c] = 0u;
    __syncthreads();
    unsigned int* h = shc + (threadIdx.x >> 6) * 3 * C;
    auto flush = [&](int pl, int tl, unsigned int len) {
        if (len == 0u) return;
        if (pl >= 0 && pl < C) atomicAdd(&h[pl], len);
        if (tl >= 0 && tl < C) atomicAdd(&h[C + tl], len);
        if (pl == tl && pl >= 0 && pl < C) atomicAdd(&h[2 * C + pl], len);
    };
    const long long nruns = (V + RUN - 1) / RUN;
    for (long long r = (long long)blockIdx.x * blockDim.x + threadIdx.x; r < nruns; r += (long long)gridDim.x * blockDim.x) {
        const long long v0 = r * RUN;
        const int cnt = (int)((V - v0) < RUN ? (V - v0) : RUN);
        int pl = -1, tl = -1; unsigned int len = 0u;
        for (int k = 0; k < cnt; ++k) {
            const long long row = (long long)n * V + v0 + k;
            const int a = (int)load_label(pred, pred_bytes, row), b = (int)load_label(truth, truth_bytes, row);
            if (a != pl || b != tl) { flush(pl, tl, len); pl = a; tl = b; len = 0u; }
            ++len;
        }
        flush(pl, tl, len);
    }
    __syncthreads();
    for (int c = threadIdx.x; c < 3 * C; c += blockDim.x) {
        const unsigned int t = shc[c] + shc[3 * C + c] + shc[6 * C + c] + shc[9 * C + c];
        const int k = c / C, cc = c % C;
        if (t) atomicAdd(&counts[((size_t)n * C + cc) * 3 + k], (unsigned long long)t);
    }
}

}

extern "C" size_t da_dice_ws_bytes(int N, long long V, int C) {
    (void)V;
    return da_align((size_t)N * kDiceBlocks * 3 * C * sizeof(double)) + da_align((size_t)3 * N * C * sizeof(float));
}

extern "C" int da_dice_fwd(const float* src, const void* labels, int label_bytes, const float* soft_target,
                           int N, long long V, int C, int softmax, int weight_type, int no_bg, float eps,
                           float* loss, float* coef, void* ws, size_t ws_bytes, void* stream) {
    if (!src || (!labels && !soft_target) || !loss || !coef || N <= 0 || N > 64 || V <= 0 || C <= 0 || C > 256) return DA_ERR_BADARG;
    if (labels && label_bytes != 1 && label_bytes != 8) return DA_ERR_BADARG;
    if (ws_bytes < da_dice_ws_bytes(N, V, C)) return DA_ERR_WS_SMALL;
    hipStream_t st = da_stream(stream);
    double* partial = (double*)ws;
    float* isc = (float*)((char*)ws + da_align((size_t)N * kDiceBlocks * 3 * C * sizeof(double)));
    const int lpv = lpv_for(C);
    int nblocks = (int)da_cdiv(V, 256); if (nblocks > kDiceBlocks) nblocks = kDiceBlocks;
    if (lpv > 0) {
        const int slots = 256 / lpv;
        hipLaunchKernelGGL(dice_partial_vec_kernel, dim3(nblocks, N), dim3(256), (size_t)3 * slots * C * sizeof(float), st,
                           src, labels, label_bytes, soft_target, V, C, lpv, softmax, partial);
    } else {
        hipLaunchKernelGGL(dice_partial_gen_kernel, dim3(nblocks, N), dim3(256), (size_t)4 * 3 * C * sizeof(float), st,
                           src, labels, label_bytes, soft_target, V, C, softmax, partial);
    }
    DA_LAUNCH_CHECK();
    hipLaunchKernelGGL(colreduce_inplace_kernel, dim3((unsigned)da_cdiv((long long)N * 3 * C * 64, 256)), dim3(256), 0, st, partial, N, nblocks, 3 * C);
    DA_LAUNCH_CHECK();
    hipLaunchKernelGGL(dice_finalize_kernel, dim3(1), dim3(256), 0, st, partial, nblocks, 1, N, C, weight_type, no_bg, eps, loss, coef, isc);
    DA_LAUNCH_CHECK();
    return 0;
}

extern "C" int da_softmax_dice_fwd(const float* src, const void* labels, int label_bytes, float* prob,
                                   int N, long long V, int C, int weight_type, int no_bg, float eps,
                                   float* loss, float* coef, void* ws, size_t ws_bytes, void* stream) {
    if (!src || !labels || !prob || !loss || !coef || N <= 0 || N > 64 || V <= 0 || C <= 0 || C > 256) return DA_ERR_BADARG;
    if (label_bytes != 1 && label_bytes != 8) return DA_ERR_BADARG;
    const int lpv = lpv_for(C);
    if (lpv <= 0) return DA_ERR_UNSUPPORTED;
    if (ws_bytes < da_dice_ws_bytes(N, V, C)) return DA_ERR_WS_SMALL;
    hipStream_t st = da_stream(stream);
    double* partial = (double*)ws;
    float* isc = (float*)((char*)ws + da_align((size_t)N * kDiceBlocks * 3 * C * sizeof(double)));
    int nblocks = (int)da_cdiv(V, 256); if (nblocks > kDiceBlocks) nblocks = kDiceBlocks;
    const int slots = 256 / lpv;
    hipLaunchKernelGGL(dice_partial_vec_kernel, dim3(nblocks, N), dim3(256), (size_t)3 * slots * C * sizeof(float), st,
                       src, labels, label_bytes, (const float*)nullptr, V, C, lpv, 1, partial, prob);
    DA_LAUNCH_CHECK();
    return da_dice_finish(partial, nblocks, N, C, weight_type, no_bg, eps, loss, coef, isc, st);
}

int da_dice_finish(double* partial, int nblocks, int N, int C, int weight_type, int no_bg, float eps,
                   float* loss, float* coef, float* isc, hipStream_t st) {
    hipLaunchKernelGGL(colreduce_inplace_kernel, dim3((unsigned)da_cdiv((long long)N * 3 * C * 64, 256)), dim3(256), 0, st, partial, N, nblocks, 3 * C);
    DA_LAUNCH_CHECK();
    hipLaunchKernelGGL(dice_finalize_kernel, dim3(1), dim3(256), 0, st, partial, nblocks, 1, N, C, weight_type, no_bg, eps, loss, coef, isc);
    DA_LAUNCH_CHECK();
    return 0;
}

extern "C" int da_dice_bwd(const float* src, const void* labels, int label_bytes, const float* soft_target,
                           const float* coef, const float* dloss, float* d_src,
                           int N, long long V, int C, int softmax, void* stream) {
    if (!src || (!labels && !soft_target) || !coef || !dloss || !d_src || N <= 0 || V <= 0 || C <= 0) return DA_ERR_BADARG;
    hipStream_t st = da_stream(stream);
    const int lpv = lpv_for(C);
    if (lpv > 0) {
        const long long total = (long long)N * V * lpv;
        hipLaunchKernelGGL(dice_bwd_vec_kernel, dim3(da_grid(total, 256)), dim3(256), 0, st, src, labels, label_bytes, soft_target, coef, dloss, d_src, N, V, C, lpv, softmax);
    } else {
        hipLaunchKernelGGL(dice_bwd_gen_kernel, dim3(da_grid((long long)N * V, 256)), dim3(256), 0, st, src, labels, label_bytes, soft_target, coef, dloss, d_src, N, V, C, softmax);
    }
    DA_LAUNCH_CHECK();
    return 0;
}

extern "C" int da_softmax_fwd(const float* x, float* y, long long M, int C, void* stream) {
    if (!x || !y || M <= 0 || C <= 0) return DA_ERR_BADARG;
    const int lpv = lpv_for(C);
    hipLaunchKernelGGL(softmax_fwd_kernel, dim3(da_grid(M * (lpv > 0 ? lpv : 1), 256)), dim3(256), 0, da_stream(stream), x, y, M, C, lpv);
    DA_LAUNCH_CHECK();
    return 0;
}

extern "C" int da_softmax_bwd(const float* dy, const float* y, float* dx, long long M, int C, void* stream) {
    if (!dy || !y || !dx || M <= 0 || C <= 0) return DA_ERR_BADARG;
    const int lpv = lpv_for(C);
    hipLaunchKernelGGL(softmax_bwd_kernel, dim3(da_grid(M * (lpv > 0 ? lpv : 1), 256)), dim3(256), 0, da_stream(stream), dy, y, dx, M, C, lpv);
    DA_LAUNCH_CHECK();
    return 0;
}

extern "C" int da_one_hot(const void* labels, int label_bytes, float* out, long long M, int C, void* stream) {
    if (!labels || !out || M <= 0 || C <= 0 || (label_bytes != 1 && label_bytes != 8)) return DA_ERR_BADARG;
    hipLaunchKernelGGL(one_hot_kernel, dim3(da_grid(M * C, 256)), dim3(256), 0, da_stream(stream), labels, label_bytes, out, M, C);
    DA_LAUNCH_CHECK();
    return 0;
}

extern "C" size_t da_ncc_ws_bytes(int N, long long V) {
    (void)V;
    return da_align((size_t)N * kBlocks * 5 * sizeof(double));
}

extern "C" int da_ncc_fwd(const float* x, const float* y, int N, long long V, float* loss, double* stats,
                          void* ws, size_t ws_bytes, void* stream) {
    if (!x || !y || !loss || !stats || N <= 0 || N > 64 || V <= 0) return DA_ERR_BADARG;
    if (ws_bytes < da_ncc_ws_bytes(N, V)) return DA_ERR_WS_SMALL;
    hipStream_t st = da_stream(stream);
    int nblocks = (int)da_cdiv(V / 4 + 1, 256 * 4); if (nblocks > kBlocks) nblocks = kBlocks; if (nblocks < 1) nblocks = 1;
    const bool aligned = ((((size_t)x | (size_t)y) & 15) == 0) && (N == 1 || (V % 4) == 0);
    if (aligned) hipLaunchKernelGGL(ncc_partial_kernel<true>, dim3(nblocks, N), dim3(256), 0, st, x, y, V, (double*)ws);
    else hipLaunchKernelGGL(ncc_partial_kernel<false>, dim3(nblocks, N), dim3(256), 0, st, x, y, V, (double*)ws);
    DA_LAUNCH_CHECK();
    hipLaunchKernelGGL(colreduce_inplace_kernel, dim3((unsigned)da_cdiv((long long)N * 5 * 64, 256)), dim3(256), 0, st, (double*)ws, N, nblocks, 5);
    DA_LAUNCH_CHECK();
    hipLaunchKernelGGL(ncc_finalize_kernel, dim3(1), dim3(64), 0, st, (const double*)ws, nblocks, 1, N, V, x, y, loss, stats);
    DA_LAUNCH_CHECK();
    return 0;
}

extern "C" int da_ncc_bwd(const float* x, const float* y, const double* stats, const float* dloss,
                          float* dx, float* dy, int N, long long V, void* stream) {
    if (!x || !y || !stats || !dloss || N <= 0 || V <= 0) return DA_ERR_BADARG;
    if (!dx && !dy) return 0;
    hipLaunchKernelGGL(ncc_bwd_kernel, dim3(da_grid(V, 256, 2048), N), dim3(256), 0, da_stream(stream), x, y, stats, dloss, dx, dy, N, V);
    DA_LAUNCH_CHECK();
    return 0;
}

extern "C" size_t da_bending_ws_bytes(int N, int D, int H, int W) {
    (void)D; (void)H; (void)W;
    return da_align((size_t)N * kBendBlocks * sizeof(double));
}

extern "C" int da_bending_fwd(const float* disp, int N, int D, int H, int W, const float* spacing3, int normalize, int norm,
                              float* loss, void* ws, size_t ws_bytes, void* stream) {
    if (!disp || !loss || N <= 0 || D < 3 || H < 3 || W < 3 || (norm != 1 && norm != 2)) return DA_ERR_BADARG;
    if (ws_bytes < da_bending_ws_bytes(N, D, H, W)) return DA_ERR_WS_SMALL;
    hipStream_t st = da_stream(stream);
    const BendK K = bending_coeffs(N, D, H, W, spacing3, normalize, norm);
    const long long total = (long long)(D - 2) * (H - 2) * (W - 2);
    int nblocks = (int)da_cdiv(total, 256); if (nblocks > kBendBlocks) nblocks = kBendBlocks; if (nblocks < 1) nblocks = 1;
    if (norm == 2) hipLaunchKernelGGL((bending_partial_kernel<false>), dim3(nblocks, N), dim3(256), 0, st, disp, D, H, W, K, (double*)ws);
    else hipLaunchKernelGGL((bending_partial_kernel<true>), dim3(nblocks, N), dim3(256), 0, st, disp, D, H, W, K, (double*)ws);
    DA_LAUNCH_CHECK();
    hipLaunchKernelGGL(scalar_finalize_kernel, dim3(1), dim3(256), 0, st, (const double*)ws, nblocks * N, loss);
    DA_LAUNCH_CHECK();
    return 0;
}

extern "C" int da_bending_bwd(const float* disp, const float* dloss, float* d_disp, int N, int D, int H, int W,
                              const float* spacing3, int normalize, int norm, void* stream) {
    if (!disp || !dloss || !d_disp || N <= 0 || D < 3 || H < 3 || W < 3 || (norm != 1 && norm != 2)) return DA_ERR_BADARG;
    const BendK K = bending_coeffs(N, D, H, W, spacing3, normalize, norm);
    const long long total = (long long)D * H * W * 3;
    if (norm == 2) hipLaunchKernelGGL((bending_bwd_kernel<false>), dim3(da_grid(total, 256, 4096), N), dim3(256), 0, da_stream(stream), disp, dloss, d_disp, D, H, W, K);
    else hipLaunchKernelGGL((bending_bwd_kernel<true>), dim3(da_grid(total, 256, 4096), N), dim3(256), 0, da_stream(stream), disp, dloss, d_disp, D, H, W, K);
    DA_LAUNCH_CHECK();
    return 0;
}

extern "C" int da_argmax_dice_counts(const float* logits, const void* truth, int label_bytes, int N, long long V, int C,
                                     unsigned long long* counts, unsigned char* pred, void* stream) {
    if (!logits || !truth || !counts || N <= 0 || V <= 0 || C <= 0 || C > 256 || (label_bytes != 1 && label_bytes != 8)) return DA_ERR_BADARG;
    const int lpv = lpv_for(C);
    const long long total = V * (lpv > 0 ? lpv : 1);
    hipLaunchKernelGGL(argmax_counts_kernel, dim3(da_grid(total, 256, 1024), N), dim3(256), (size_t)3 * C * sizeof(unsigned int), da_stream(stream),
                       logits, truth, label_bytes, V, C, lpv, counts, pred);
    DA_LAUNCH_CHECK();
    return 0;
}

extern "C" int da_label_overlap_counts(const void* pred, int pred_bytes, const void* truth, int truth_bytes, int N, long long V, int C,
                                       unsigned long long* counts, void* stream) {
    if (!pred || !truth || !counts || N <= 0 || V <= 0 || C <= 0 || C > 1024 || (pred_bytes != 1 && pred_bytes != 8) || (truth_bytes != 1 && truth_bytes != 8))
        return DA_ERR_BADARG;
    hipLaunchKernelGGL(label_overlap_counts_kernel, dim3(da_grid((V + 15) / 16, 256, 1024), N), dim3(256), (size_t)4 * 3 * C * sizeof(unsigned int),
                       da_stream(stream), pred, pred_bytes, truth, truth_bytes, V, C, counts);
    DA_LAUNCH_CHECK();
    return 0;
}
```

include/deepatlas_hip.h:

```cpp
#ifndef DEEPATLAS_HIP_H
#define DEEPATLAS_HIP_H

#include <stddef.h>
#include <stdint.h>

#ifdef __cplusplus
extern "C" {
#endif

#define DA_ERR_BADARG   (-1)
#define DA_ERR_WS_SMALL (-2)
#define DA_ERR_UNSUPPORTED (-3)

int  da_version(void);
int  da_device_info(int* cu_count, int* wave_size, size_t* hbm_bytes, char* arch, int arch_len);

int da_w_oik_to_tio(const float* w_oik, float* w_tio, int Cout, int Cin, int K3, void* stream);
int da_w_tio_to_oik(const float* w_tio, float* w_oik, int Cout, int Cin, int K3, void* stream);
int da_w_iok_to_tio(const float* w_iok, float* w_tio, int Cin, int Cout, int K3, void* stream);
int da_w_tio_to_iok(const float* w_tio, float* w_iok, int Cin, int Cout, int K3, void* stream);
int da_w_iok_flip_to_tio(const float* w_iok, float* w_tio, int Cin, int Cout, int K3, void* stream);
int da_w_tio_to_iok_flip(const float* w_tio, float* w_iok, int Cin, int Cout, int K3, void* stream);
int da_w_tio_to_oik_acc(const float* w_tio, float* w_oik, int Cout, int Cin, int K3, void* stream);
int da_w_tio_to_iok_acc(const float* w_tio, float* w_iok, int Cin, int Cout, int K3, void* stream);
int da_w_tio_to_iok_flip_acc(const float* w_tio, float* w_iok, int Cin, int Cout, int K3, void* stream);

size_t da_conv3d_k3_ws_bytes(int N, int D, int H, int W, int Cin, int Cout, int stride);
int da_conv3d_k3_fwd(const float* in1, int C1, const float* in2, int C2,
                     const float* w_tio, const float* bias, float* out,
                     int N, int D, int H, int W, int Cout, int stride, float act_slope,
                     void* ws, size_t ws_bytes, void* stream);
int da_conv3d_k3_fwd_bnstats(const float* in1, int C1, const float* in2, int C2,
                             const float* w_tio, const float* bias, float* out,
                             int N, int D, int H, int W, int Cout, int stride,
                             double* stats_partial, int stats_capacity, int* stats_nparts,
                             void* ws, size_t ws_bytes, void* stream);
int da_conv3d_k3_dgrad(const float* dy, const float* w_tio, float* dx1, int C1, float* dx2, int C2,
                       int N, int D, int H, int W, int Cout, int stride,
                       void* ws, size_t ws_bytes, void* stream);
int da_conv3d_k3_wgrad(const float* in1, int C1, const float* in2, int C2, const float* dy,
                       float* dw_tio, float* dbias,
                       int N, int D, int H, int W, int Cout, int stride,
                       void* ws, size_t ws_bytes, void* stream);

int da_conv3d_k3_fwd_pro(const float* in1, int C1, const float* pro1_scale, const float* pro1_shift, float pro1_slope,
                         const float* in2, int C2, const float* pro2_scale, const float* pro2_shift, float pro2_slope,
                         const float* w_tio, const float* bias, float* out,
                         int N, int D, int H, int W, int Cout, float act_slope,
                         double* stats_partial, int stats_capacity, int* stats_nparts,
                         void* ws, size_t ws_bytes, void* stream);
int da_conv3d_k3_wgrad_pro(const float* in1, int C1, const float* pro1_scale, const float* pro1_shift, float pro1_slope,
                           const float* in2, int C2, const float* pro2_scale, const float* pro2_shift, float pro2_slope,
                           const float* dy, float* dw_tio,
                           int N, int D, int H, int W, int Cout,
                           void* ws, size_t ws_bytes, void* stream);

int da_upconv3d_k3_supported(int C1, int C2, int Cout);
size_t da_upconv3d_k3_ws_bytes(int N, int Dc, int Hc, int Wc, int Cin, int Cout);
int da_upconv3d_k3_fwd(const float* s1, int C1, const float* s2, int C2, const float* w_tio, const float* bias, float* out,
                       int N, int Dc, int Hc, int Wc, int Cout, float act_slope, void* ws, size_t ws_bytes, void* stream);
int da_upconv3d_k3_dgrad(const float* dy, const float* w_tio, float* dx1, int C1, float* dx2, int C2,
                         int N, int Dc, int Hc, int Wc, int Cout, void* ws, size_t ws_bytes, void* stream);
int da_upconv3d_k3_wgrad(const float* s1, int C1, const float* s2, int C2, const float* dy, float* dw_tio,
                         int N, int Dc, int Hc, int Wc, int Cout, void* ws, size_t ws_bytes, void* stream);

int da_set_conv_direct(int on);

int da_set_matrix_bf16(int on);
int da_set_matrix_mode(int mode);

size_t da_pointwise_ws_bytes(int ntaps, int Cin, int Cout);
int da_conv1x1_fwd(const float* in, const float* w_io, const float* bias, float* out,
                   long long M, int Cin, int Cout, void* ws, size_t ws_bytes, void* stream);
int da_conv1x1_fwd_pro(const float* in, const float* pro_scale, const float* pro_shift, float pro_slope,
                       const float* w_io, const float* bias, float* out,
                       long long M, int Cin, int Cout, void* ws, size_t ws_bytes, void* stream);
int da_conv1x1_wgrad_pro(const float* in, const float* pro_scale, const float* pro_shift, float pro_slope,
                         const float* dy, float* dw_io, float* dbias,
                         long long M, int Cin, int Cout, void* ws, size_t ws_bytes, void* stream);
int da_conv1x1_dgrad(const float* dy, const float* w_io, float* dx, long long M, int Cin, int Cout,
                     void* ws, size_t ws_bytes, void* stream);
size_t da_conv1x1_wgrad_ws_bytes(long long M, int Cin, int Cout);
int da_conv1x1_wgrad(const float* in, const float* dy, float* dw_io, float* dbias,
                     long long M, int Cin, int Cout, void* ws, size_t ws_bytes, void* stream);

int da_deconv_k2s2_fwd(const float* in, const float* w_tio, const float* bias, float* out,
                       int N, int D, int H, int W, int Cin, int Cout, void* ws, size_t ws_bytes, void* stream);
int da_deconv_k2s2_fwd_bnstats(const float* in, const float* w_tio, const float* bias, float* out,
                               int N, int D, int H, int W, int Cin, int Cout,
                               double* stats_partial, int stats_capacity, int* stats_nparts,
                               void* ws, size_t ws_bytes, void* stream);
int da_deconv_k2s2_dgrad(const float* dy, const float* w_tio, float* dx,
                         int N, int D, int H, int W, int Cin, int Cout, void* ws, size_t ws_bytes, void* stream);
size_t da_deconv_k2s2_bn_bwd_ws_bytes(int N, int D, int H, int W, int Cin, int Cout);
int da_deconv_k2s2_bn_bwd(const float* gout, const float* y, const float* mean, const float* rstd, const float* scale, const float* shift, float act_slope,
                          const float* in, const float* w_tio, float* dx, float* dw_tio, float* dbias, float* dgamma, float* dbeta,
                          int N, int D, int H, int W, int Cin, int Cout, const double* pre, int pre_n,
                          void* ws, size_t ws_bytes, void* stream);
size_t da_deconv_k2s2_wgrad_ws_bytes(int N, int D, int H, int W, int Cin, int Cout);
int da_deconv_k2s2_wgrad(const float* in, const float* dy, float* dw_tio, float* dbias,
                         int N, int D, int H, int W, int Cin, int Cout,
                         void* ws, size_t ws_bytes, void* stream);

size_t da_bn_ws_bytes(long long M, int C);
int da_bn_train_stats(const float* x, long long M, int C, const float* gamma, const float* beta,
                      float eps, float momentum, float* running_mean, float* running_var,
                      float* mean, float* rstd, float* scale, float* shift,
                      void* ws, size_t ws_bytes, void* stream);
int da_bn_train_stats_from_partials(const double* partial, int nparts, long long M, int C,
                                    const float* gamma, const float* beta, float eps, float momentum,
                                    float* running_mean, float* running_var,
                                    float* mean, float* rstd, float* scale, float* shift, void* stream);
int da_bn_eval_affine(const float* gamma, const float* beta, const float* running_mean, const float* running_var,
                      float eps, int C, float* mean, float* rstd, float* scale, float* shift, void* stream);
int da_bn_act_fwd(const float* x, const float* scale, const float* shift, float act_slope, float* y,
                  long long M, int C, void* stream);
int da_bn_act_bwd(const float* dy, const float* x, const float* mean, const float* rstd, const float* gamma,
                  const float* scale, const float* shift, float act_slope, int train,
                  float* dx, float* dgamma, float* dbeta, long long M, int C,
                  void* ws, size_t ws_bytes, void* stream);
int da_bn_act_bwd_dbias(const float* dy, const float* x, const float* mean, const float* rstd,
                        const float* scale, const float* shift, float act_slope, int train,
                        float* dx, float* dgamma, float* dbeta, float* dxsum, long long M, int C,
                        void* ws, size_t ws_bytes, void* stream);
int da_bn_act_bwd_dbias_pre(const float* dy, const float* x, const float* mean, const float* rstd,
                            const float* scale, const float* shift, float act_slope, int train,
                            float* dx, float* dgamma, float* dbeta, float* dxsum, long long M, int C,
                            const double* pre, int pre_n, void* ws, size_t ws_bytes, void* stream);
int da_act_bwd(const float* dy, const float* y, float act_slope, float* dx, long long numel, void* stream);
int da_act_bwd_add_dbias(const float* g1, const float* g2, const float* y, float act_slope, float* dx, float* dbias,
                         long long M, int C, void* ws, size_t ws_bytes, void* stream);
int da_colsum(const float* x, long long M, int C, float* out, void* ws, size_t ws_bytes, void* stream);
int da_act_bwd_add_partial(const float* g1, const float* g2, const float* y, float act_slope, float* dx,
                           long long M, int C, void* partial, size_t partial_bytes, int* nparts, void* stream);
int da_colsum_finish(const void* partial, int nparts, int C, float* out, int accumulate, void* stream);

int da_maxpool2_fwd(const float* x, float* y, int N, int D, int H, int W, int C, void* stream);
int da_maxpool2_fwd_pro(const float* x, const float* pro_scale, const float* pro_shift, float pro_slope, float* act, float* y,
                        int N, int D, int H, int W, int C, void* stream);
int da_maxpool2_bwd(const float* dy, const float* x, float* dx, int N, int D, int H, int W, int C, void* stream);
int da_maxpool2_bwd_add(const float* dy, const float* x, const float* gskip, float* dx, int N, int D, int H, int W, int C, void* stream);
int da_maxpool2_bwd_bst(const float* dy, const float* x_raw, const float* gskip, float* dx, int N, int D, int H, int W, int C,
                        const float* stats4, float slope, double* bst, int bst_cap, int* bst_n, void* stream);

int da_upsample_nearest_fwd(const float* x, float* y, int N, int D, int H, int W, int C,
                            int Do, int Ho, int Wo, void* stream);
int da_upsample_nearest_bwd(const float* dy, float* dx, int N, int D, int H, int W, int C,
                            int Do, int Ho, int Wo, void* stream);

int da_warp_fwd(const float* src, const float* disp, float* deform, float* out,
                int N, int D, int H, int W, int C, void* stream);
int da_warp_bwd(const float* dout, const float* src, const float* disp, float* d_disp, float* d_src,
                int N, int D, int H, int W, int C, void* stream);
int da_warp_labels_fwd(const void* labels, int label_bytes, const float* disp, float* out,
                       int N, int D, int H, int W, int C, void* stream);
int da_warp_labels_bwd(const float* dout, const void* labels, int label_bytes, const float* disp, float* d_disp,
                       int N, int D, int H, int W, int C, void* stream);
int da_identity_grid(float* out, int D, int H, int W, int normalize, void* stream);
size_t da_label_warp_dice_ws_bytes(int N, int C);
int da_label_warp_dice_fwd(const void* lab_m, int lab_m_bytes, const void* lab_t, int lab_t_bytes, const float* disp,
                           int N, int D, int H, int W, int C, int weight_type, int no_bg, float eps,
                           float* loss, float* coef , void* ws, size_t ws_bytes, void* stream);
int da_label_warp_dice_bwd(const void* lab_m, int lab_m_bytes, const void* lab_t, int lab_t_bytes, const float* disp,
                           const float* coef, const float* dloss, float* d_disp, int N, int D, int H, int W, int C, void* stream);
int da_softmax_dice_fwd(const float* src, const void* labels, int label_bytes, float* prob,
                        int N, long long V, int C, int weight_type, int no_bg, float eps,
                        float* loss, float* coef , void* ws , size_t ws_bytes, void* stream);
size_t da_warp_dice_ws_bytes(int N, int C);
int da_warp_dice_fwd(const float* src, const float* disp, const void* lab_t, int lab_t_bytes,
                     int N, int D, int H, int W, int C, int weight_type, int no_bg, float eps,
                     float* loss, float* coef , void* ws, size_t ws_bytes, void* stream);
int da_warp_adjoint_labels(const void* lab_t, int lab_t_bytes, const float* disp, float* A, float* B,
                           int N, int D, int H, int W, int C, void* stream);
int da_seg_anat_dlogits(const float* prob, const void* lab_m, int lab_m_bytes, const float* A, const float* B, float* dlogits,
                        const float* coef_sup, const float* coef_anat, const float* dloss_sup, const float* dloss_anat,
                        int N, long long V, int C, void* stream);
size_t da_softwarp_dice_ws_bytes(int N, int C);
int da_softwarp_dice_fwd(const void* lab_m, int lab_m_bytes, const float* disp, const float* dense, int role,
                         int N, int D, int H, int W, int C, int weight_type, int no_bg, float eps,
                         float* loss, float* coef , void* ws, size_t ws_bytes, void* stream);
int da_softwarp_dice_bwd_disp(const void* lab_m, int lab_m_bytes, const float* disp, const float* prob, const float* coef, const float* dloss,
                              float* d_disp, int N, int D, int H, int W, int C, void* stream);
int da_softwarp_dice_bwd_logits(const void* lab_m, int lab_m_bytes, const float* disp, const float* logits, const float* coef, const float* dloss,
                                float* dlogits, int N, int D, int H, int W, int C, void* stream);
size_t da_warp_bwd_dsrc_det_ws_bytes(int N, int D, int H, int W, int C);
int da_warp_bwd_dsrc_det(const float* dout, const float* disp, float* d_src, int N, int D, int H, int W, int C,
                         void* ws, size_t ws_bytes, void* stream);

size_t da_dice_ws_bytes(int N, long long V, int C);
int da_dice_fwd(const float* src, const void* labels, int label_bytes, const float* soft_target,
                int N, long long V, int C, int softmax, int weight_type, int no_bg, float eps,
                float* loss, float* coef, void* ws, size_t ws_bytes, void* stream);
int da_dice_bwd(const float* src, const void* labels, int label_bytes, const float* soft_target,
                const float* coef, const float* dloss, float* d_src,
                int N, long long V, int C, int softmax, void* stream);
int da_softmax_fwd(const float* x, float* y, long long M, int C, void* stream);
int da_softmax_bwd(const float* dy, const float* y, float* dx, long long M, int C, void* stream);
int da_one_hot(const void* labels, int label_bytes, float* out, long long M, int C, void* stream);

size_t da_head_dice_ws_bytes(int N, long long V, int Cin, int C);
int da_head_dice_fwd(const float* x, const float* pro_scale, const float* pro_shift, float pro_slope,
                     const float* w_io, const float* bias, const void* labels, int label_bytes,
                     int N, long long V, int Cin, int C, int weight_type, int no_bg, float eps,
                     float* loss, float* coef, void* ws, size_t ws_bytes, void* stream);
int da_head_dice_bwd(const float* x, const float* pro_scale, const float* pro_shift, float pro_slope,
                     const float* w_io, const float* bias, const void* labels, int label_bytes,
                     const float* coef, const float* dloss, float* dx, float* dw_io, float* dbias,
                     int N, long long V, int Cin, int C, void* ws, size_t ws_bytes, void* stream);
int da_head_dice_bwd_bst(const float* x, const float* pro_scale, const float* pro_shift, float pro_slope, const float* pro_mean,
                         const float* w_io, const float* bias, const void* labels, int label_bytes,
                         const float* coef, const float* dloss, float* dx, float* dw_io, float* dbias,
                         int N, long long V, int Cin, int C, double* bst, int bst_cap, int* bst_n, void* ws, size_t ws_bytes, void* stream);

int da_conv3d_k3_dgrad_bst(const float* dy, const float* w_tio, float* dx1, int C1, float* dx2, int C2, int N, int D, int H, int W, int Cout,
                           const float* y, const float* stats4, float slope, double* bst, int bst_cap, int* bst_n,
                           void* ws, size_t ws_bytes, void* stream);

size_t da_conv3d_k3_pack_bytes(int N, int D, int H, int W, int Cin, int Cout);
int da_conv3d_k3_prepack(const float* w_tio, int C1, int C2, int Cout, int dgrad, int N, int D, int H, int W,
                         void* b0, size_t n0, void* b1, size_t n1, int* used, void* stream);
void da_conv3d_k3_use_prepacked(const float* w_tio, const void* b0, size_t n0, const void* b1, size_t n1);
int da_conv3d_k3_prepack_many(int n, const float* const* w_tio, const int* C1, const int* C2, const int* Cout, const int* dgrad,
                              const int* N, const int* D, const int* H, const int* W,
                              void* const* b0, const size_t* n0, void* const* b1, const size_t* n1, int* used, void* stream);

size_t da_ncc_ws_bytes(int N, long long V);
int da_ncc_fwd(const float* x, const float* y, int N, long long V, float* loss, double* stats ,
               void* ws, size_t ws_bytes, void* stream);
int da_ncc_bwd(const float* x, const float* y, const double* stats, const float* dloss,
               float* dx, float* dy, int N, long long V, void* stream);

size_t da_bending_ws_bytes(int N, int D, int H, int W);
int da_bending_fwd(const float* disp, int N, int D, int H, int W, const float* spacing3, int normalize, int norm,
                   float* loss, void* ws, size_t ws_bytes, void* stream);
int da_bending_bwd(const float* disp, const float* dloss, float* d_disp, int N, int D, int H, int W,
                   const float* spacing3, int normalize, int norm, void* stream);

size_t da_xent_ws_bytes(void);
int da_xent_fwd(const float* logits, const void* labels, int label_bytes, const float* soft_target, const float* alpha,
                long long M, int C, int mode, int softmax, float gamma, long long ignore_index, int reduction,
                float* loss, float* denom, void* ws, size_t ws_bytes, void* stream);
int da_xent_bwd(const float* logits, const void* labels, int label_bytes, const float* soft_target, const float* alpha,
                const float* dloss, const float* denom, float* dlogits, long long M, int C, int mode, int softmax, float gamma,
                long long ignore_index, void* stream);

int da_conv_k2s2_fwd(const float* x, const float* w_tio, const float* bias, float* y,
                     int N, int D, int H, int W, int Cin, int Cout, void* ws, size_t ws_bytes, void* stream);
int da_conv_k2s2_dgrad(const float* dy, const float* w_tio, float* dx,
                       int N, int D, int H, int W, int Cin, int Cout, void* ws, size_t ws_bytes, void* stream);
size_t da_conv_k2s2_wgrad_ws_bytes(int N, int D, int H, int W, int Cin, int Cout);
int da_conv_k2s2_wgrad(const float* x, const float* dy, float* dw_toi, float* dbias,
                       int N, int D, int H, int W, int Cin, int Cout, void* ws, size_t ws_bytes, void* stream);
int da_upsample_trilinear2_fwd(const float* x, float* y, int N, int D, int H, int W, int C, void* stream);
int da_upsample_trilinear2_bwd(const float* dy, float* dx, int N, int D, int H, int W, int C, void* stream);

int da_clamp01_to_f32(const void* src, int src_dtype, float* dst, long long n, void* stream);
int da_crop3d(const void* src, void* dst, int elem_bytes, long long C, int D, int H, int W,
              int d0, int h0, int w0, int Do, int Ho, int Wo, void* stream);
int da_partition_tiles(const void* vol, void* tiles, int elem_bytes, int D, int H, int W, const int* tile3, const int* overlap3, void* stream);
int da_assemble_tiles(const void* tiles, void* vol, int elem_bytes, int D, int H, int W, const int* tile3, const int* overlap3, int vote, void* stream);

int da_synth_volume(float* img, unsigned char* labels, int N, int D, int H, int W, int n_classes, int mode, float noise,
                    unsigned int seed, int sample0, void* stream);

#define DA_AUG_MAX_GRID_POINTS 2048
int da_spatial_resample(const float* img, float* img_out, int C, int interp,
                        const void* labels, void* labels_out, int label_bytes,
                        const float* affine, const float* coef, int order, int gx, int gy, int gz,
                        int N, int D, int H, int W, void* stream);

size_t da_lncc_ws_bytes(int N, int D, int H, int W, int F, int dil, int stride);
int da_lncc_fwd(const float* I, const float* J, int N, int D, int H, int W, int F, int dil, int stride, float eps,
                float* loss, float* sums, void* ws, size_t ws_bytes, void* stream);
int da_lncc_bwd(const float* I, const float* J, const float* sums, const float* dloss, float* dI, float* dJ,
                int N, int D, int H, int W, int F, int dil, int stride, float eps, void* ws, size_t ws_bytes, void* stream);

#define DA_MI_STATS_FLOATS 1096
size_t da_mi_ws_bytes(int N, long long V, int bins);
int da_mi_fwd(const float* x, const float* y, int N, long long V, int bins, float vmin, float vmax, float sigma_ratio,
              float* loss, float* stats, void* ws, size_t ws_bytes, void* stream);
int da_mi_bwd(const float* x, const float* y, const float* stats, const float* dloss, float* dx, float* dy,
              int N, long long V, int bins, float vmin, float vmax, float sigma_ratio, void* stream);

size_t da_gradloss_ws_bytes(int N, int D, int H, int W);
int da_gradloss_fwd(const float* disp, int N, int D, int H, int W, const float* spacing3, int normalize, int norm,
                    float* loss, void* ws, size_t ws_bytes, void* stream);
int da_gradloss_bwd(const float* disp, const float* dloss, float* d_disp, int N, int D, int H, int W,
                    const float* spacing3, int normalize, int norm, void* stream);

int da_argmax_dice_counts(const float* logits, const void* truth, int label_bytes, int N, long long V, int C,
                          unsigned long long* counts, unsigned char* pred, void* stream);

int da_label_overlap_counts(const void* pred, int pred_bytes, const void* truth, int truth_bytes, int N, long long V, int C,
                            unsigned long long* counts, void* stream);

int da_warp_labels_nearest_counts(const void* lab_m, int m_bytes, const void* lab_t, int t_bytes, const float* disp,
                                  int N, int D, int H, int W, int C, unsigned long long* counts, unsigned char* warped, void* stream);
size_t da_jacobian_det_ws_bytes(int N, int D, int H, int W);
int da_jacobian_det(const float* disp, int N, int D, int H, int W, double* stats , float* det_out,
                    void* ws, size_t ws_bytes, void* stream);
size_t da_jacdet_penalty_ws_bytes(int N, int D, int H, int W);
int da_jacdet_penalty_fwd(const float* disp, int N, int D, int H, int W, float eps, int power, float* loss, double* stats ,
                          float* det, void* ws, size_t ws_bytes, void* stream);
int da_jacdet_penalty_bwd(const float* disp, const float* det, const float* dloss, float* d_disp, int N, int D, int H, int W,
                          float eps, int power, void* stream);
size_t da_invcons_ws_bytes(int N, int D, int H, int W);
int da_invcons_fwd(const float* disp_a, const float* disp_b, int N, int D, int H, int W, float* loss, double* stats ,
                   float* resid , void* ws, size_t ws_bytes, void* stream);
int da_invcons_bwd(const float* disp_a, const float* disp_b, const float* resid, const float* dloss, float* d_disp_a, float* d_disp_b,
                   int N, int D, int H, int W, int deterministic, void* ws, size_t ws_bytes, void* stream);
int da_affine_warp_fwd(const float* src, const float* theta, float* out, int N, int D, int H, int W, int C, void* stream);
size_t da_affine_warp_ws_bytes(int N, int D, int H, int W);
int da_affine_warp_bwd_theta(const float* g, const float* src, const float* theta, float* d_theta , int N, int D, int H, int W,
                             int C, void* ws, size_t ws_bytes, void* stream);
int da_affine_compose_disp(const float* theta, const float* disp , float* out ,
                           int N, int D, int H, int W, void* stream);
size_t da_field_invert_ws_bytes(int N, int D, int H, int W);
int da_field_invert(const float* disp, float* out, unsigned char* iters , int N, int D, int H, int W, int max_iters,
                    float tol_vox, double* stats , void* ws, size_t ws_bytes, void* stream);
size_t da_field_points_ws_bytes(int N, int P);
int da_field_transport_points(const float* disp, const float* points, float* out, int N, int D, int H, int W, int P, int inverse,
                              int max_iters, float tol_vox, double* stats , void* ws, size_t ws_bytes, void* stream);
int da_label_fusion_vote(const void* labels, int label_bytes, long long label_sample_stride, const float* disp,
                         const float* w_atlas, const float* w_voxel, int N, int K, int D, int H, int W,
                         unsigned char* fused, float* conf, void* stream);
size_t da_local_msd_weights_ws_bytes(int N, int K, int D, int H, int W);
int da_local_msd_weights(const float* warped, const float* target, int N, int K, int D, int H, int W, int radius, float beta,
                         float* weights, void* ws, size_t ws_bytes, void* stream);

int da_adam_step(float* p, const float* g, float* m, float* v, long long n,
                 float lr, float beta1, float beta2, float eps, int step, float grad_scale, void* stream);

int da_adam_host_state(float lr, float beta1, float beta2, float eps, int step, float grad_scale, float* state6_host);
int da_adam_step_dev(float* p, const float* g, float* m, float* v, long long n, float* state6, void* stream);

int da_cast_f32_to_bf16(const float* x, void* y, long long numel, void* stream);
int da_cast_bf16_to_f32(const void* x, float* y, long long numel, void* stream);
int da_bn_train_stats_bf16(const void* x, long long M, int C, const float* gamma, const float* beta,
                           float eps, float momentum, float* running_mean, float* running_var,
                           float* mean, float* rstd, float* scale, float* shift, void* ws, size_t ws_bytes, void* stream);
int da_bn_act_fwd_bf16(const void* x, const float* scale, const float* shift, float act_slope, void* y, long long M, int C, void* stream);
int da_bn_act_bwd_dbias_bf16(const void* dy, const void* x, const float* mean, const float* rstd,
                             const float* scale, const float* shift, float act_slope, int train,
                             void* dx, float* dgamma, float* dbeta, float* dxsum, long long M, int C,
                             void* ws, size_t ws_bytes, void* stream);
int da_act_bwd_bf16(const void* dy, const void* y, float act_slope, void* dx, long long numel, void* stream);
int da_act_bwd_add_dbias_bf16(const void* g1, const void* g2, const void* y, float act_slope, void* dx, float* dbias,
                              long long M, int C, void* ws, size_t ws_bytes, void* stream);
int da_act_bwd_add_partial_bf16(const void* g1, const void* g2, const void* y, float act_slope, void* dx,
                                long long M, int C, void* partial, size_t partial_bytes, int* nparts, void* stream);
int da_colsum_bf16(const void* x, long long M, int C, float* out, void* ws, size_t ws_bytes, void* stream);
int da_maxpool2_fwd_bf16(const void* x, void* y, int N, int D, int H, int W, int C, void* stream);
int da_maxpool2_fwd_pro_bf16(const void* x, const float* pro_scale, const float* pro_shift, float pro_slope, void* act, void* y,
                             int N, int D, int H, int W, int C, void* stream);
int da_maxpool2_bwd_bf16(const void* dy, const void* x, void* dx, int N, int D, int H, int W, int C, void* stream);
int da_maxpool2_bwd_add_bf16(const void* dy, const void* x, const void* gskip, void* dx, int N, int D, int H, int W, int C, void* stream);
int da_upsample_nearest_fwd_bf16(const void* x, void* y, int N, int D, int H, int W, int C, int Do, int Ho, int Wo, void* stream);
int da_upsample_nearest_bwd_bf16(const void* dy, void* dx, int N, int D, int H, int W, int C, int Do, int Ho, int Wo, void* stream);
int da_conv3d_k3_fwd_bf16(const void* in1, int C1, const void* in2, int C2, const float* w_tio, const float* bias, void* out,
                          int N, int D, int H, int W, int Cout, int stride, float act_slope,
                          void* ws, size_t ws_bytes, void* stream, unsigned bf16_mask);
int da_conv3d_k3_fwd_bnstats_bf16(const void* in1, int C1, const void* in2, int C2, const float* w_tio, const float* bias, void* out,
                                  int N, int D, int H, int W, int Cout, int stride,
                                  double* stats_partial, int stats_capacity, int* stats_nparts,
                                  void* ws, size_t ws_bytes, void* stream, unsigned bf16_mask);
int da_conv3d_k3_fwd_pro_bf16(const void* in1, int C1, const float* pro1_scale, const float* pro1_shift, float pro1_slope,
                              const void* in2, int C2, const float* pro2_scale, const float* pro2_shift, float pro2_slope,
                              const float* w_tio, const float* bias, void* out,
                              int N, int D, int H, int W, int Cout, float act_slope,
                              double* stats_partial, int stats_capacity, int* stats_nparts,
                              void* ws, size_t ws_bytes, void* stream, unsigned bf16_mask);
int da_conv3d_k3_wgrad_pro_bf16(const void* in1, int C1, const float* pro1_scale, const float* pro1_shift, float pro1_slope,
                                const void* in2, int C2, const float* pro2_scale, const float* pro2_shift, float pro2_slope,
                                const void* dy, float* dw_tio, int N, int D, int H, int W, int Cout,
                                void* ws, size_t ws_bytes, void* stream, unsigned bf16_mask);
int da_conv3d_k3_dgrad_bf16(const void* dy, const float* w_tio, void* dx1, int C1, void* dx2, int C2,
                            int N, int D, int H, int W, int Cout, int stride, void* ws, size_t ws_bytes, void* stream, unsigned bf16_mask);
int da_conv3d_k3_wgrad_bf16(const void* in1, int C1, const void* in2, int C2, const void* dy, float* dw_tio, float* dbias,
                            int N, int D, int H, int W, int Cout, int stride, void* ws, size_t ws_bytes, void* stream, unsigned bf16_mask);
int da_deconv_k2s2_fwd_bf16(const void* in, const float* w_tio, const float* bias, void* out,
                            int N, int D, int H, int W, int Cin, int Cout, void* ws, size_t ws_bytes, void* stream);
int da_deconv_k2s2_fwd_bnstats_bf16(const void* in, const float* w_tio, const float* bias, void* out,
                                    int N, int D, int H, int W, int Cin, int Cout,
                                    double* stats_partial, int stats_capacity, int* stats_nparts, void* ws, size_t ws_bytes, void* stream);
int da_deconv_k2s2_dgrad_bf16(const void* dy, const float* w_tio, void* dx,
                              int N, int D, int H, int W, int Cin, int Cout, void* ws, size_t ws_bytes, void* stream);
int da_deconv_k2s2_wgrad_bf16(const void* in, const void* dy, float* dw_tio, float* dbias,
                              int N, int D, int H, int W, int Cin, int Cout, void* ws, size_t ws_bytes, void* stream);
int da_conv1x1_fwd_bf16(const void* in, const float* w_io, const float* bias, float* out,
                        long long M, int Cin, int Cout, void* ws, size_t ws_bytes, void* stream);
int da_conv1x1_fwd_pro_bf16(const void* in, const float* pro_scale, const float* pro_shift, float pro_slope,
                            const float* w_io, const float* bias, float* out, long long M, int Cin, int Cout, void* ws, size_t ws_bytes, void* stream);
int da_conv1x1_dgrad_bf16(const float* dy, const float* w_io, void* dx, long long M, int Cin, int Cout, void* ws, size_t ws_bytes, void* stream);
int da_conv1x1_wgrad_bf16(const void* in, const float* dy, float* dw_io, float* dbias,
                          long long M, int Cin, int Cout, void* ws, size_t ws_bytes, void* stream);
int da_conv1x1_wgrad_pro_bf16(const void* in, const float* pro_scale, const float* pro_shift, float pro_slope,
                              const float* dy, float* dw_io, float* dbias, long long M, int Cin, int Cout, void* ws, size_t ws_bytes, void* stream);
int da_head_dice_fwd_bf16(const void* x, const float* pro_scale, const float* pro_shift, float pro_slope,
                          const float* w_io, const float* bias, const void* labels, int label_bytes,
                          int N, long long V, int Cin, int C, int weight_type, int no_bg, float eps,
                          float* loss, float* coef, void* ws, size_t ws_bytes, void* stream);
int da_head_dice_bwd_bf16(const void* x, const float* pro_scale, const float* pro_shift, float pro_slope,
                          const float* w_io, const float* bias, const void* labels, int label_bytes,
                          const float* coef, const float* dloss, void* dx, float* dw_io, float* dbias,
                          int N, long long V, int Cin, int C, void* ws, size_t ws_bytes, void* stream);

#ifdef __cplusplus
}
#endif
#endif
```

Before: 100.2 volumes/s.

## Restructure head-dice kernels with persistent chunk scheduling and direct weight loads

Reworks the fused head+softmax+Dice forward and backward kernels. A persistent grid now walks voxel chunks across batch samples, and the per-wave tile size is a template parameter. Weight pre-packing is dropped in favour of reading w_io directly, and the separate partial-reduce plus memcpy steps are replaced by one reduce kernel that writes dw/dbias. The softmax normalisation is folded into the accumulation, and the dice finalize kernel is parallelised across threads. The intent is to cut small-kernel launch count and ALU work, in exchange for more complex scheduling and different reduction ordering.

Result: no change. 99.99 volumes/s (-0.2%).

```diff
diff --git a/deepatlas_amd/_native.py b/deepatlas_amd/_native.py
--- a/deepatlas_amd/_native.py
+++ b/deepatlas_amd/_native.py
@@ -108,6 +108,7 @@
     'da_head_dice_fwd': (I, [P, P, P, F, P, P, P, I, I, LL, I, I, I, I, F, P, P, P, SZ, P]),
     'da_head_dice_bwd': (I, [P, P, P, F, P, P, P, I, P, P, P, P, P, I, LL, I, I, P, SZ, P]),
     'da_head_dice_bwd_bst': (I, [P, P, P, F, P, P, P, P, I, P, P, P, P, P, I, LL, I, I, P, I, P, P, SZ, P]),
+    'da_head_dice_grid': (I, [I, I, I, I, P]),
     'da_ncc_ws_bytes': (SZ, [I, LL]),
     'da_ncc_fwd': (I, [P, P, I, LL, P, P, P, SZ, P]),
     'da_ncc_bwd': (I, [P, P, P, P, P, P, I, LL, P]),
diff --git a/deepatlas_amd/csrc/headdice.hip b/deepatlas_amd/csrc/headdice.hip
--- a/deepatlas_amd/csrc/headdice.hip
+++ b/deepatlas_amd/csrc/headdice.hip
@@ -5,12 +5,14 @@
 namespace {
 
 constexpr int kHdBlocks = 1024;
-constexpr int MT = 4;
+constexpr int kHdChunk = 256;
 constexpr float kLog2e = 1.44269504088896341f;
+constexpr int hd_mt_fwd(int KC) { return 2; }
+constexpr int hd_mt(int KC) { return KC == 1 ? 2 : 4; }
 
 struct HdP {
     const float* x; const float* ps; const float* pt; float pslope;
-    const float* wp_fwd; const float* wp_bwd; const float* bias;
+    const float* w_io; const float* bias;
     const void* labels; int label_bytes;
     long long V; int N, K, C;
     double* partial;
@@ -20,53 +22,34 @@
 };
 
 __device__ __forceinline__ float hd_act01(float z, float s) { return fmaxf(z, z * s); }
-__device__ __forceinline__ long long hd_label(const void* labels, int label_bytes, long long i) {
-    return label_bytes == 1 ? (long long)((const unsigned char*)labels)[i] : ((const long long*)labels)[i];
-}
-
-__global__ void hd_pack_kernel(const float* __restrict__ w, float* __restrict__ wp, int K, int N, int transposed) {
-    const int KC = K / 16, NT = N / 16;
-    const int total = NT * KC * 256;
-    for (int idx = blockIdx.x * blockDim.x + threadIdx.x; idx < total; idx += gridDim.x * blockDim.x) {
-        const int m = idx & 3, lane = (idx >> 2) & 63;
-        int rest = idx >> 8;
-        const int c = rest % KC; const int n = rest / KC;
-        const int k = 16 * c + 4 * (lane >> 4) + m, j = 16 * n + (lane & 15);
-        wp[idx] = transposed ? w[(size_t)j * K + k] : w[(size_t)k * N + j];
-    }
-}
-
-typedef float f2 __attribute__((ext_vector_type(2)));
-__device__ __forceinline__ f2 hd_lo(f32x4 v) { return __builtin_shufflevector(v, v, 0, 1); }
-__device__ __forceinline__ f2 hd_hi(f32x4 v) { return __builtin_shufflevector(v, v, 2, 3); }
-__device__ __forceinline__ f2 hd_bc(float x) { return (f2){x, x}; }
-
-template <int KC, typename T>
+__device__ __forceinline__ float hd_max3(float a, float b, float c) { return fmaxf(fmaxf(a, b), c); }
+
+template <int MT>
+__device__ __forceinline__ int hd_last(const HdP& p, long long vbase) { return (int)min(p.V - 1 - vbase, (long long)(64 * MT)); }
+template <int KC, int MT, typename T>
 __device__ __forceinline__ void hd_load(const HdP& p, const T* __restrict__ xs, long long vbase, int i, int g, float4 (&a)[MT][KC]) {
+    const T* xb = xs + vbase * (KC * 16);
+    const int last = hd_last<MT>(p, vbase);
 #pragma unroll
     for (int t = 0; t < MT; ++t) {
-        const long long vox = min(vbase + t * 16 + i, p.V - 1);
-#pragma unroll
-        for (int c = 0; c < KC; ++c) a[t][c] = da_ldq(xs, (vox * p.K + 16 * c + 4 * g) >> 2);
-    }
-}
+        const int o = min(t * 16 + i, last);
+#pragma unroll
+        for (int c = 0; c < KC; ++c) a[t][c] = da_ldq(xb, (long long)(o * (KC * 4) + 4 * c + g));
+    }
+}
+template <int MT>
 __device__ __forceinline__ void hd_labels(const HdP& p, long long lbase, long long vbase, int i, int g, int (&rel)[MT]) {
-#pragma unroll
-    for (int t = 0; t < MT; ++t) rel[t] = (int)((const unsigned char*)p.labels)[(lbase + min(vbase + t * 16 + i, p.V - 1)) * p.label_bytes];
-}
-__device__ __forceinline__ int hd_rel(const HdP& p, int lab, long long vox, int g) { return (vox < p.V ? lab : -1000) - 4 * g; }
-template <int NT>
-__device__ __forceinline__ void hd_mask(int rel, f2 (&mk)[NT][2]) {
-#pragma unroll
-    for (int n = 0; n < NT; ++n) {
-        mk[n][0] = (f2){rel == 16 * n ? 1.f : 0.f, rel == 16 * n + 1 ? 1.f : 0.f};
-        mk[n][1] = (f2){rel == 16 * n + 2 ? 1.f : 0.f, rel == 16 * n + 3 ? 1.f : 0.f};
-    }
-}
-
-template <int KC, int NT, typename T = float>
+    const int lsh = p.label_bytes == 8 ? 3 : 0, last = hd_last<MT>(p, vbase);
+    const unsigned char* lb = (const unsigned char*)p.labels + ((lbase + vbase) << lsh);
+#pragma unroll
+    for (int t = 0; t < MT; ++t) rel[t] = (int)lb[(long long)(min(t * 16 + i, last) << lsh)];
+}
+__device__ __forceinline__ int hd_rel(int lab, bool valid, int g) { return (valid ? lab : -1000) - 4 * g; }
+
+template <int KC, int NT, int MT, typename T = float>
 __device__ __forceinline__ void hd_probs(const HdP& p, long long vbase, int i, int g, const float4 (&psc)[KC], const float4 (&psf)[KC],
-                                         const float4 (&wf)[NT][KC], const float (&bv)[NT][4], float4 (&a)[MT][KC], f32x4 (&acc)[MT][NT]) {
+                                         const float4 (&wf)[NT][KC], const float (&bv)[NT][4], float4 (&a)[MT][KC], f32x4 (&acc)[MT][NT], float (&inv)[MT]) {
+    const int last = hd_last<MT>(p, vbase);
     if (p.ps) {
 #pragma unroll
         for (int c = 0; c < KC; ++c) {
@@ -104,46 +87,41 @@
     }
 #pragma unroll
     for (int t = 0; t < MT; ++t) {
-        const bool valid = vbase + t * 16 + i < p.V;
-        float m = acc[t][0][0];
-#pragma unroll
-        for (int n = 0; n < NT; ++n)
-#pragma unroll
-            for (int reg = 0; reg < 4; ++reg) m = fmaxf(m, acc[t][n][reg]);
+        const bool valid = t * 16 + i <= last;
+        float m = hd_max3(acc[t][0][0], acc[t][0][1], acc[t][0][2]);
+        m = fmaxf(m, acc[t][0][3]);
+#pragma unroll
+        for (int n = 1; n < NT; ++n) { m = hd_max3(m, acc[t][n][0], acc[t][n][1]); m = hd_max3(m, acc[t][n][2], acc[t][n][3]); }
         m = da_rows_max(m);
-        f2 s2 = (f2){0.f, 0.f};
+        float s = 0.f;
 #pragma unroll
         for (int n = 0; n < NT; ++n) {
 #pragma unroll
             for (int reg = 0; reg < 4; ++reg) acc[t][n][reg] = __builtin_amdgcn_exp2f(acc[t][n][reg] - m);
-            s2 += hd_lo(acc[t][n]) + hd_hi(acc[t][n]);
-        }
-        const float s = da_rows_sum(s2.x + s2.y);
-        const f2 inv = hd_bc(valid ? __builtin_amdgcn_rcpf(s) : 0.f);
-#pragma unroll
-        for (int n = 0; n < NT; ++n) {
-            const f2 lo = hd_lo(acc[t][n]) * inv, hi = hd_hi(acc[t][n]) * inv;
-            acc[t][n] = (f32x4){lo.x, lo.y, hi.x, hi.y};
-        }
-    }
-}
-
+            s += (acc[t][n][0] + acc[t][n][1]) + (acc[t][n][2] + acc[t][n][3]);
+        }
+        s = da_rows_sum(s);
+        inv[t] = valid ? __builtin_amdgcn_rcpf(s) : 0.f;
+    }
+}
+
+template <int KC, int NT>
+__device__ __forceinline__ void hd_weights(const HdP& p, int i, int g, float4 (&wf)[NT][KC]) {
+    constexpr int C = NT * 16;
+#pragma unroll
+    for (int n = 0; n < NT; ++n)
+#pragma unroll
+        for (int c = 0; c < KC; ++c) {
+            const float* w = p.w_io + (size_t)(16 * c + 4 * g) * C + 16 * n + i;
+            wf[n][c] = make_float4(w[0] * kLog2e, w[C] * kLog2e, w[2 * C] * kLog2e, w[3 * C] * kLog2e);
+        }
+}
 template <int NT>
 __device__ __forceinline__ void hd_bias(const HdP& p, int g, float (&bv)[NT][4]) {
 #pragma unroll
     for (int n = 0; n < NT; ++n)
 #pragma unroll
         for (int reg = 0; reg < 4; ++reg) bv[n][reg] = p.bias ? p.bias[16 * n + 4 * g + reg] * kLog2e : 0.f;
-}
-template <int KC, int NT>
-__device__ __forceinline__ void hd_weights(const HdP& p, int lane, float4 (&wf)[NT][KC]) {
-#pragma unroll
-    for (int n = 0; n < NT; ++n)
-#pragma unroll
-        for (int c = 0; c < KC; ++c) {
-            const float4 w = reinterpret_cast<const float4*>(p.wp_fwd)[(n * KC + c) * 64 + lane];
-            wf[n][c] = make_float4(w.x * kLog2e, w.y * kLog2e, w.z * kLog2e, w.w * kLog2e);
-        }
 }
 template <int KC>
 __device__ __forceinline__ void hd_prologue(const HdP& p, int g, float4 (&psc)[KC], float4 (&psf)[KC]) {
@@ -153,78 +131,106 @@
         psf[c] = p.ps ? *reinterpret_cast<const float4*>(p.pt + 16 * c + 4 * g) : make_float4(0.f, 0.f, 0.f, 0.f);
     }
 }
-
-template <int KC, int NT, typename T = float>
+struct HdPos { int n; long long l; int s; };
+__device__ __forceinline__ HdPos hd_start(long long b, long long cps, int N) {
+    HdPos q{0, b, 0};
+    while (q.l >= cps && q.n < N) { q.l -= cps; ++q.n; }
+    return q;
+}
+template <int MT>
+__device__ __forceinline__ HdPos hd_next(HdPos q, long long grid, long long cps, int N, long long V) {
+    if constexpr (64 * MT < kHdChunk) {
+        if (q.s + 1 < kHdChunk / (64 * MT) && q.l * kHdChunk + (q.s + 1) * (64 * MT) < V) { ++q.s; return q; }
+    }
+    q.s = 0; q.l += grid;
+    while (q.l >= cps && q.n < N) { q.l -= cps; ++q.n; }
+    return q;
+}
+
+template <int KC, int NT, int MT, typename T = float>
 __global__ void __launch_bounds__(256) head_dice_fwd_kernel(HdP p) {
-    __shared__ double sred[4][3][NT * 16];
-    const int lane = threadIdx.x & 63, wave = threadIdx.x >> 6;
+    constexpr int C = NT * 16, CV = 64 * MT;
+    __shared__ double sred[4][3][C];
+    const int lane = threadIdx.x & 63, wave = __builtin_amdgcn_readfirstlane(threadIdx.x >> 6);
     const int i = lane & 15, g = lane >> 4;
-    const int n_s = blockIdx.y;
-    const T* xs = reinterpret_cast<const T*>(p.x) + (long long)n_s * p.V * p.K;
-    const long long lbase = (long long)n_s * p.V;
     float4 wf[NT][KC]; float bv[NT][4]; float4 psc[KC], psf[KC];
     hd_bias<NT>(p, g, bv);
-    hd_weights<KC, NT>(p, lane, wf);
+    hd_weights<KC, NT>(p, i, g, wf);
     hd_prologue<KC>(p, g, psc, psf);
-    f2 sI[NT][2], sS[NT][2], sT[NT][2];
-#pragma unroll
-    for (int n = 0; n < NT; ++n)
-#pragma unroll
-        for (int h = 0; h < 2; ++h) sI[n][h] = sS[n][h] = sT[n][h] = (f2){0.f, 0.f};
-    const long long nchunks = (p.V + 255) / 256;
+    const long long cps = (p.V + kHdChunk - 1) / kHdChunk;
+    HdPos cur = hd_start(blockIdx.x, cps, p.N);
     float4 an[MT][KC]; int reln[MT];
-    if ((long long)blockIdx.x < nchunks) { hd_load<KC, T>(p, xs, (long long)blockIdx.x * 256 + wave * 64, i, g, an); hd_labels(p, lbase, (long long)blockIdx.x * 256 + wave * 64, i, g, reln); }
-    for (long long cb = blockIdx.x; cb < nchunks; cb += gridDim.x) {
-        const long long vbase = cb * 256 + wave * 64;
-        float4 a[MT][KC]; f32x4 acc[MT][NT]; int rel[MT];
-#pragma unroll
-        for (int t = 0; t < MT; ++t) {
-            rel[t] = hd_rel(p, reln[t], vbase + t * 16 + i, g);
-#pragma unroll
-            for (int c = 0; c < KC; ++c) a[t][c] = an[t][c];
-        }
-        { const long long vn = min(cb + (long long)gridDim.x, nchunks - 1) * 256 + wave * 64; hd_load<KC, T>(p, xs, vn, i, g, an); hd_labels(p, lbase, vn, i, g, reln); }
-        hd_probs<KC, NT, T>(p, vbase, i, g, psc, psf, wf, bv, a, acc);
-#pragma unroll
-        for (int t = 0; t < MT; ++t) {
-            f2 mk[NT][2];
-            hd_mask<NT>(rel[t], mk);
-#pragma unroll
-            for (int n = 0; n < NT; ++n) {
-                const f2 lo = hd_lo(acc[t][n]), hi = hd_hi(acc[t][n]);
-                sS[n][0] += lo; sS[n][1] += hi;
-                sI[n][0] += lo * mk[n][0]; sI[n][1] += hi * mk[n][1];
-                sT[n][0] += mk[n][0]; sT[n][1] += mk[n][1];
+    auto fetch = [&](HdPos q) {
+        const long long vb = q.l * kHdChunk + q.s * CV + wave * (16 * MT);
+        hd_load<KC, MT, T>(p, reinterpret_cast<const T*>(p.x) + (long long)q.n * p.V * p.K, vb, i, g, an);
+        hd_labels<MT>(p, (long long)q.n * p.V, vb, i, g, reln);
+    };
+    if (cur.n < p.N) fetch(cur);
+    for (int n_s = 0; n_s < p.N; ++n_s) {
+        float sI[NT][4], sS[NT][4]; int cT[NT][4];
+#pragma unroll
+        for (int n = 0; n < NT; ++n)
+#pragma unroll
+            for (int reg = 0; reg < 4; ++reg) { sI[n][reg] = 0.f; sS[n][reg] = 0.f; cT[n][reg] = 0; }
+        const bool any = cur.n == n_s;
+        while (cur.n == n_s) {
+            const long long vbase = cur.l * kHdChunk + cur.s * CV + wave * (16 * MT);
+            const int last = hd_last<MT>(p, vbase);
+            float4 a[MT][KC]; f32x4 acc[MT][NT]; int rel[MT]; float inv[MT];
+#pragma unroll
+            for (int t = 0; t < MT; ++t) {
+                rel[t] = hd_rel(reln[t], t * 16 + i <= last, g);
+#pragma unroll
+                for (int c = 0; c < KC; ++c) a[t][c] = an[t][c];
             }
-        }
-    }
-#pragma unroll
-    for (int n = 0; n < NT; ++n)
-#pragma unroll
-        for (int reg = 0; reg < 4; ++reg) {
-            double a0 = (double)sI[n][reg >> 1][reg & 1], a1 = (double)sS[n][reg >> 1][reg & 1], a2 = (double)sT[n][reg >> 1][reg & 1];
-#pragma unroll
-            for (int o = 1; o < 16; o <<= 1) { a0 += __shfl_xor(a0, o); a1 += __shfl_xor(a1, o); a2 += __shfl_xor(a2, o); }
-            if (i == 0) { const int c = 16 * n + 4 * g + reg; sred[wave][0][c] = a0; sred[wave][1][c] = a1; sred[wave][2][c] = a2; }
-        }
-    __syncthreads();
-    for (int idx = threadIdx.x; idx < 3 * p.C; idx += blockDim.x) {
-        const int k = idx / p.C, c = idx % p.C;
-        p.partial[(((size_t)n_s * gridDim.x + blockIdx.x) * 3 + k) * p.C + c] = (sred[0][k][c] + sred[1][k][c]) + (sred[2][k][c] + sred[3][k][c]);
-    }
-}
-
-template <int KC, int NT, typename T = float>
-__global__ void __launch_bounds__(256) head_dice_bwd_kernel(HdP p) {
-    constexpr int K = KC * 16, C = NT * 16, LDX = K + 4, LDD = C + 4;
+            const HdPos nxt = hd_next<MT>(cur, gridDim.x, cps, p.N, p.V);
+            fetch(nxt.n < p.N ? nxt : cur);
+            hd_probs<KC, NT, MT, T>(p, vbase, i, g, psc, psf, wf, bv, a, acc, inv);
+#pragma unroll
+            for (int t = 0; t < MT; ++t)
+#pragma unroll
+                for (int n = 0; n < NT; ++n)
+#pragma unroll
+                    for (int reg = 0; reg < 4; ++reg) {
+                        const bool hit = rel[t] == 16 * n + reg;
+                        const float e = acc[t][n][reg];
+                        sS[n][reg] = fmaf(e, inv[t], sS[n][reg]);
+                        sI[n][reg] = fmaf(e, hit ? inv[t] : 0.f, sI[n][reg]);
+                        cT[n][reg] += hit ? 1 : 0;
+                    }
+            cur = nxt;
+        }
+        if (any) {
+#pragma unroll
+            for (int n = 0; n < NT; ++n)
+#pragma unroll
+                for (int reg = 0; reg < 4; ++reg) {
+                    double a0 = (double)sI[n][reg], a1 = (double)sS[n][reg], a2 = (double)cT[n][reg];
+#pragma unroll
+                    for (int o = 1; o < 16; o <<= 1) { a0 += __shfl_xor(a0, o); a1 += __shfl_xor(a1, o); a2 += __shfl_xor(a2, o); }
+                    if (i == 0) { const int c = 16 * n + 4 * g + reg; sred[wave][0][c] = a0; sred[wave][1][c] = a1; sred[wave][2][c] = a2; }
+                }
+        }
+        __syncthreads();
+        for (int idx = threadIdx.x; idx < 3 * C; idx += blockDim.x) {
+            const int k = idx / C, c = idx % C;
+            p.partial[(((size_t)n_s * gridDim.x + blockIdx.x) * 3 + k) * C + c] = any ? (sred[0][k][c] + sred[1][k][c]) + (sred[2][k][c] + sred[3][k][c]) : 0.0;
+        }
+        __syncthreads();
+    }
+}
+
+template <int KC, int NT, int MT, typename T = float>
+__global__ void __launch_bounds__(256) __attribute__((amdgpu_waves_per_eu(MT == 2 ? 3 : 1))) head_dice_bwd_kernel(HdP p) {
+    constexpr int K = KC * 16, C = NT * 16, LDX = K + 4, LDD = C + 4, WV = 16 * MT, CV = 64 * MT;
     extern __shared__ __attribute__((aligned(16))) float lds[];
-    const int lane = threadIdx.x & 63, wave = threadIdx.x >> 6;
+    const int lane = threadIdx.x & 63, wave = __builtin_amdgcn_readfirstlane(threadIdx.x >> 6);
     const int i = lane & 15, g = lane >> 4;
-    float* xl = lds + wave * (64 * LDX + 64 * LDD);
-    float* dl = xl + 64 * LDX;
+    float* xl = lds + wave * (WV * LDX + WV * LDD);
+    float* dl = xl + WV * LDX;
     float4 wf[NT][KC]; float bv[NT][4]; float4 psc[KC], psf[KC];
     hd_bias<NT>(p, g, bv);
-    hd_weights<KC, NT>(p, lane, wf);
+    hd_weights<KC, NT>(p, i, g, wf);
     hd_prologue<KC>(p, g, psc, psf);
     float wd[KC][NT][4];
 #pragma unroll
@@ -232,74 +238,86 @@
 #pragma unroll
         for (int n = 0; n < NT; ++n)
 #pragma unroll
-            for (int reg = 0; reg < 4; ++reg) wd[c][n][reg] = p.wp_bwd[(size_t)(16 * c + i) * C + 16 * n + 4 * g + reg];
+            for (int reg = 0; reg < 4; ++reg) wd[c][n][reg] = p.w_io[(size_t)(16 * c + i) * C + 16 * n + 4 * g + reg];
     const float gl = p.dloss[0];
     f32x4 wacc[KC][NT];
 #pragma unroll
     for (int c = 0; c < KC; ++c)
 #pragma unroll
         for (int n = 0; n < NT; ++n) wacc[c][n] = (f32x4){0.f, 0.f, 0.f, 0.f};
-    f2 db[NT][2];
-#pragma unroll
-    for (int n = 0; n < NT; ++n) db[n][0] = db[n][1] = (f2){0.f, 0.f};
+    float db[NT][4];
+#pragma unroll
+    for (int n = 0; n < NT; ++n)
+#pragma unroll
+        for (int reg = 0; reg < 4; ++reg) db[n][reg] = 0.f;
     const bool bst = KC == 1 && p.bst != nullptr;
     float4 bsc = make_float4(0.f, 0.f, 0.f, 0.f), bsf = bsc, bmu = bsc;
     float bs1[4] = {0.f, 0.f, 0.f, 0.f}, bs2[4] = {0.f, 0.f, 0.f, 0.f};
-    if (bst) { bsc = *reinterpret_cast<const float4*>(p.ps + 4 * g); bsf = *reinterpret_cast<const float4*>(p.pt + 4 * g); bmu = *reinterpret_cast<const float4*>(p.pmean + 4 * g); }
-    const long long chunks_per_sample = (p.V + 255) / 256, nchunks = chunks_per_sample * p.N;
+    if (bst) { bsc = psc[0]; bsf = psf[0]; bmu = *reinterpret_cast<const float4*>(p.pmean + 4 * g); }
+    const long long cps = (p.V + kHdChunk - 1) / kHdChunk;
+    HdPos cur = hd_start(blockIdx.x, cps, p.N);
     float4 an[MT][KC]; int reln[MT];
-    auto fetch = [&](long long cb) {
-        const int n_s = (int)(cb / chunks_per_sample);
-        const long long vbase = (cb - (long long)n_s * chunks_per_sample) * 256 + wave * 64;
-        hd_load<KC, T>(p, reinterpret_cast<const T*>(p.x) + (long long)n_s * p.V * p.K, vbase, i, g, an);
-        hd_labels(p, (long long)n_s * p.V, vbase, i, g, reln);
+    auto fetch = [&](HdPos q) {
+        const long long vb = q.l * kHdChunk + q.s * CV + wave * WV;
+        hd_load<KC, MT, T>(p, reinterpret_cast<const T*>(p.x) + (long long)q.n * p.V * p.K, vb, i, g, an);
+        hd_labels<MT>(p, (long long)q.n * p.V, vb, i, g, reln);
     };
-    if ((long long)blockIdx.x < nchunks) fetch(blockIdx.x);
-    for (long long cb = blockIdx.x; cb < nchunks; cb += gridDim.x) {
-        const int n_s = (int)(cb / chunks_per_sample);
-        const long long vbase = (cb - (long long)n_s * chunks_per_sample) * 256 + wave * 64;
+    if (cur.n < p.N) fetch(cur);
+    float k01[NT][4], k1[NT][4];
+    int n_k = -1;
+    while (cur.n < p.N) {
+        const int n_s = cur.n;
+        const long long vbase = cur.l * kHdChunk + cur.s * CV + wave * WV;
+        const int last = hd_last<MT>(p, vbase);
         const T* xs = reinterpret_cast<const T*>(p.x) + (long long)n_s * p.V * p.K;
         T* dxs = reinterpret_cast<T*>(p.dx) + (long long)n_s * p.V * p.K;
-        const float* c0 = p.coef + (size_t)n_s * p.C;
-        const float* c1 = p.coef + (size_t)(p.N + n_s) * p.C;
-        float4 a[MT][KC]; f32x4 acc[MT][NT]; int rel[MT];
+        if (n_s != n_k) {
+            const float* c0 = p.coef + (size_t)n_s * C;
+            const float* c1 = p.coef + (size_t)(p.N + n_s) * C;
+#pragma unroll
+            for (int n = 0; n < NT; ++n)
+#pragma unroll
+                for (int reg = 0; reg < 4; ++reg) {
+                    const float v0 = c0[16 * n + 4 * g + reg], v1 = c1[16 * n + 4 * g + reg];
+                    k01[n][reg] = gl * (v0 + v1); k1[n][reg] = gl * v1;
+                }
+            n_k = n_s;
+        }
+        float4 a[MT][KC]; f32x4 acc[MT][NT]; int rel[MT]; float inv[MT];
 #pragma unroll
         for (int t = 0; t < MT; ++t) {
-            rel[t] = hd_rel(p, reln[t], vbase + t * 16 + i, g);
+            rel[t] = hd_rel(reln[t], t * 16 + i <= last, g);
 #pragma unroll
             for (int c = 0; c < KC; ++c) a[t][c] = an[t][c];
         }
-        fetch(min(cb + (long long)gridDim.x, nchunks - 1));
-        hd_probs<KC, NT, T>(p, vbase, i, g, psc, psf, wf, bv, a, acc);
+        const HdPos nxt = hd_next<MT>(cur, gridDim.x, cps, p.N, p.V);
+        fetch(nxt.n < p.N ? nxt : cur);
+        hd_probs<KC, NT, MT, T>(p, vbase, i, g, psc, psf, wf, bv, a, acc, inv);
 #pragma unroll
         for (int t = 0; t < MT; ++t)
 #pragma unroll
             for (int c = 0; c < KC; ++c) *reinterpret_cast<float4*>(xl + (t * 16 + i) * LDX + 16 * c + 4 * g) = a[t][c];
-        f2 k0[NT][2], k1[NT][2];
-#pragma unroll
-        for (int n = 0; n < NT; ++n)
-#pragma unroll
-            for (int h = 0; h < 2; ++h) {
-                k0[n][h] = (f2){c0[16 * n + 4 * g + 2 * h], c0[16 * n + 4 * g + 2 * h + 1]};
-                k1[n][h] = (f2){c1[16 * n + 4 * g + 2 * h], c1[16 * n + 4 * g + 2 * h + 1]};
-            }
 #pragma unroll
         for (int t = 0; t < MT; ++t) {
-            f2 mk[NT][2], gg[NT][2], pr[NT][2], dot2 = (f2){0.f, 0.f};
-            hd_mask<NT>(rel[t], mk);
+            float gg[NT][4], dot = 0.f;
+#pragma unroll
+            for (int n = 0; n < NT; ++n)
+#pragma unroll
+                for (int reg = 0; reg < 4; ++reg) {
+                    gg[n][reg] = rel[t] == 16 * n + reg ? k01[n][reg] : k1[n][reg];
+                    dot = fmaf(gg[n][reg], acc[t][n][reg], dot);
+                }
+            const float q = (da_rows_sum(dot) * inv[t]) * inv[t];
 #pragma unroll
             for (int n = 0; n < NT; ++n) {
-                pr[n][0] = hd_lo(acc[t][n]); pr[n][1] = hd_hi(acc[t][n]);
-#pragma unroll
-                for (int h = 0; h < 2; ++h) { gg[n][h] = k0[n][h] * mk[n][h] + k1[n][h]; dot2 += gg[n][h] * pr[n][h]; }
-            }
-            const f2 dot = hd_bc(da_rows_sum(dot2.x + dot2.y)), gl2 = hd_bc(gl);
-#pragma unroll
-            for (int n = 0; n < NT; ++n) {
-                const f2 d0 = (gl2 * pr[n][0]) * (gg[n][0] - dot), d1 = (gl2 * pr[n][1]) * (gg[n][1] - dot);
-                db[n][0] += d0; db[n][1] += d1;
-                acc[t][n] = (f32x4){d0.x, d0.y, d1.x, d1.y};
-                *reinterpret_cast<float4*>(dl + (t * 16 + i) * LDD + 16 * n + 4 * g) = make_float4(d0.x, d0.y, d1.x, d1.y);
+                f32x4 d;
+#pragma unroll
+                for (int reg = 0; reg < 4; ++reg) {
+                    d[reg] = acc[t][n][reg] * fmaf(gg[n][reg], inv[t], -q);
+                    db[n][reg] += d[reg];
+                }
+                acc[t][n] = d;
+                *reinterpret_cast<float4*>(dl + (t * 16 + i) * LDD + 16 * n + 4 * g) = make_float4(d[0], d[1], d[2], d[3]);
             }
         }
 #pragma unroll
@@ -313,13 +331,13 @@
                 for (int reg = 0; reg < 4; ++reg)
 #pragma unroll
                     for (int c = 0; c < KC; ++c) dacc[c] = __builtin_amdgcn_mfma_f32_16x16x4f32(wd[c][n][reg], acc[t][n][reg], dacc[c], 0, 0, 0);
-            const long long vox = vbase + t * 16 + i;
-            if (vox < p.V) {
+            if (t * 16 + i <= last) {
+                const long long q0 = (long long)((t * 16 + i) * (KC * 4) + g);
 #pragma unroll
                 for (int c = 0; c < KC; ++c)
-                    da_stq_nt(dxs, (vox * p.K + 16 * c + 4 * g) >> 2, make_float4(dacc[c][0], dacc[c][1], dacc[c][2], dacc[c][3]));
+                    da_stq_nt(dxs + vbase * K, q0 + 4 * c, make_float4(dacc[c][0], dacc[c][1], dacc[c][2], dacc[c][3]));
                 if (bst) {
-                    const float4 xr = da_ldq(xs, (vox * p.K + 4 * g) >> 2);
+                    const float4 xr = da_ldq(xs + vbase * K, q0);
                     const float xv[4] = {xr.x, xr.y, xr.z, xr.w}, scv[4] = {bsc.x, bsc.y, bsc.z, bsc.w}, sfv[4] = {bsf.x, bsf.y, bsf.z, bsf.w}, muv[4] = {bmu.x, bmu.y, bmu.z, bmu.w};
 #pragma unroll
                     for (int j = 0; j < 4; ++j) {
@@ -331,7 +349,7 @@
         }
         __builtin_amdgcn_wave_barrier();
 #pragma unroll 4
-        for (int s = 0; s < 16; ++s) {
+        for (int s = 0; s < 4 * MT; ++s) {
             float av[KC], bw[NT];
 #pragma unroll
             for (int c = 0; c < KC; ++c) av[c] = xl[(4 * s + g) * LDX + 16 * c + i];
@@ -343,6 +361,7 @@
                 for (int n = 0; n < NT; ++n) wacc[c][n] = __builtin_amdgcn_mfma_f32_16x16x4f32(av[c], bw[n], wacc[c][n], 0, 0, 0);
         }
         __builtin_amdgcn_wave_barrier();
+        cur = nxt;
     }
     __syncthreads();
     float* red = lds;
@@ -361,7 +380,7 @@
             for (int n = 0; n < NT; ++n)
 #pragma unroll
                 for (int reg = 0; reg < 4; ++reg) {
-                    float d = db[n][reg >> 1][reg & 1];
+                    float d = db[n][reg];
 #pragma unroll
                     for (int o = 1; o < 16; o <<= 1) d += __shfl_xor(d, o);
                     const int cidx = K * C + 16 * n + 4 * g + reg;
@@ -388,6 +407,53 @@
             p.bst[((size_t)blockIdx.x * 2 + k) * 16 + c] = (dred[(0 * 2 + k) * 16 + c] + dred[(1 * 2 + k) * 16 + c]) + (dred[(2 * 2 + k) * 16 + c] + dred[(3 * 2 + k) * 16 + c]);
         }
     }
+}
+
+__global__ void __launch_bounds__(256) hd_reduce_kernel(const float* __restrict__ partial, int nparts, int KCC, int O, float* __restrict__ dw, float* __restrict__ dbias) {
+    __shared__ double sh[16][17];
+    const int ol = threadIdx.x & 15, sl = threadIdx.x >> 4;
+    const int o = blockIdx.x * 16 + ol;
+    double s0 = 0.0, s1 = 0.0, s2 = 0.0, s3 = 0.0;
+    if (o < O) {
+        int b = sl;
+        for (; b + 48 < nparts; b += 64) {
+            s0 += (double)partial[(size_t)b * O + o]; s1 += (double)partial[(size_t)(b + 16) * O + o];
+            s2 += (double)partial[(size_t)(b + 32) * O + o]; s3 += (double)partial[(size_t)(b + 48) * O + o];
+        }
+        for (; b < nparts; b += 16) s0 += (double)partial[(size_t)b * O + o];
+    }
+    sh[sl][ol] = (s0 + s1) + (s2 + s3);
+    __syncthreads();
+    if (sl == 0 && o < O) {
+        double t = 0.0;
+#pragma unroll
+        for (int k = 0; k < 16; ++k) t += sh[k][ol];
+        if (o < KCC) dw[o] = (float)t;
+        else if (dbias) dbias[o - KCC] = (float)t;
+    }
+}
+
+template <auto Kern>
+static int hd_resident(size_t shm) {
+    static const int nb = [shm]() {
+        int dev = 0, cus = 0, per = 0;
+        if (hipGetDevice(&dev) != hipSuccess || hipDeviceGetAttribute(&cus, hipDeviceAttributeMultiprocessorCount, dev) != hipSuccess ||
+            hipOccupancyMaxActiveBlocksPerMultiprocessor(&per, reinterpret_cast<const void*>(Kern), 256, shm) != hipSuccess || per < 1 || cus < 1) return -1;
+        const long long g = (long long)per * cus;
+        return (int)(g > kHdBlocks ? kHdBlocks : g);
+    }();
+    return nb;
+}
+template <int KC, int NT>
+constexpr size_t hd_bwd_lds() { return (size_t)4 * (16 * hd_mt(KC) * (KC * 16 + 4) + 16 * hd_mt(KC) * (NT * 16 + 4)) * sizeof(float); }
+template <int KC, int NT, typename T> static int hd_grid_fwd() { return hd_resident<head_dice_fwd_kernel<KC, NT, hd_mt_fwd(KC), T>>(0); }
+template <int KC, int NT, typename T> static int hd_grid_bwd() { return hd_resident<head_dice_bwd_kernel<KC, NT, hd_mt(KC), T>>(hd_bwd_lds<KC, NT>()); }
+template <typename T>
+static int hd_grid(int Cin, int C, bool bwd) {
+    if (Cin == 16 && C == 32) return bwd ? hd_grid_bwd<1, 2, T>() : hd_grid_fwd<1, 2, T>();
+    if (Cin == 16 && C == 16) return bwd ? hd_grid_bwd<1, 1, T>() : hd_grid_fwd<1, 1, T>();
+    if (Cin == 64 && C == 32) return bwd ? hd_grid_bwd<4, 2, T>() : hd_grid_fwd<4, 2, T>();
+    return bwd ? hd_grid_bwd<4, 1, T>() : hd_grid_fwd<4, 1, T>();
 }
 
 static bool hd_shape_ok(int K, int C) { return (K == 16 || K == 64) && (C == 16 || C == 32); }
@@ -404,14 +470,13 @@
 
 template <int KC, int NT, typename T>
 static int hd_launch_fwd(const HdP& p, int nblocks, hipStream_t st) {
-    hipLaunchKernelGGL((head_dice_fwd_kernel<KC, NT, T>), dim3(nblocks, p.N), dim3(256), 0, st, p);
+    hipLaunchKernelGGL((head_dice_fwd_kernel<KC, NT, hd_mt_fwd(KC), T>), dim3(nblocks), dim3(256), 0, st, p);
     DA_LAUNCH_CHECK();
     return 0;
 }
 template <int KC, int NT, typename T>
 static int hd_launch_bwd(const HdP& p, int nblocks, hipStream_t st) {
-    const size_t shm = (size_t)4 * (64 * (KC * 16 + 4) + 64 * (NT * 16 + 4)) * sizeof(float);
-    return da_launch_lds<head_dice_bwd_kernel<KC, NT, T>>(dim3(nblocks), dim3(256), shm, st, p);
+    return da_launch_lds<head_dice_bwd_kernel<KC, NT, hd_mt(KC), T>>(dim3(nblocks), dim3(256), hd_bwd_lds<KC, NT>(), st, p);
 }
 
 template <typename T>
@@ -424,16 +489,14 @@
     if (!hd_shape_ok(Cin, C) || (pro_scale && pro_slope >= 1.f)) return DA_ERR_UNSUPPORTED;
     if (ws_bytes < da_head_dice_ws_bytes(N, V, Cin, C)) return DA_ERR_WS_SMALL;
     hipStream_t st = da_stream(stream);
-    float* wp = (float*)ws;
-    hipLaunchKernelGGL(hd_pack_kernel, dim3(da_grid(Cin * C, 256, 64)), dim3(256), 0, st, w_io, wp, Cin, C, 0);
-    DA_LAUNCH_CHECK();
     char* rest = (char*)ws + da_align((size_t)2 * Cin * C * sizeof(float));
     double* partial = (double*)rest;
     float* isc = (float*)(rest + da_align((size_t)N * kHdBlocks * 3 * C * sizeof(double)));
-    int nblocks = (int)da_cdiv(V, 256 * 2); if (nblocks > kHdBlocks) nblocks = kHdBlocks; if (nblocks < 1) nblocks = 1;
+    const int nblocks = hd_grid<T>(Cin, C, false);
+    if (nblocks < 1) return (int)hipErrorUnknown;
     HdP p;
     p.x = x; p.ps = pro_scale; p.pt = pro_shift; p.pslope = pro_scale ? (pro_slope < 0.f ? 1.f : pro_slope) : 1.f;
-    p.wp_fwd = wp; p.wp_bwd = nullptr; p.bias = bias; p.labels = labels; p.label_bytes = label_bytes;
+    p.w_io = w_io; p.bias = bias; p.labels = labels; p.label_bytes = label_bytes;
     p.V = V; p.N = N; p.K = Cin; p.C = C; p.partial = partial; p.coef = nullptr; p.dloss = nullptr; p.dx = nullptr; p.wpartial = nullptr; p.pmean = nullptr; p.bst = nullptr;
     int rc;
     if (Cin == 16 && C == 32) rc = hd_launch_fwd<1, 2, T>(p, nblocks, st);
@@ -468,34 +531,27 @@
     if (!hd_shape_ok(Cin, C) || (pro_scale && pro_slope >= 1.f)) return DA_ERR_UNSUPPORTED;
     if (ws_bytes < da_head_dice_ws_bytes(N, V, Cin, C)) return DA_ERR_WS_SMALL;
     hipStream_t st = da_stream(stream);
-    float* wpf = (float*)ws;
-    const float* wpb = w_io;
-    hipLaunchKernelGGL(hd_pack_kernel, dim3(da_grid(Cin * C, 256, 64)), dim3(256), 0, st, w_io, wpf, Cin, C, 0);
-    DA_LAUNCH_CHECK();
     char* rest = (char*)ws + da_align((size_t)2 * Cin * C * sizeof(float));
     float* wpartial = (float*)rest;
     const int O = Cin * C + C;
-    float* folded = (float*)(rest + da_align((size_t)kHdBlocks * O * sizeof(float)));
-    const long long nchunks = da_cdiv(V, 256) * N;
-    int nblocks = (int)(nchunks < kHdBlocks ? nchunks : kHdBlocks); if (nblocks < 1) nblocks = 1;
+    const int nblocks = hd_grid<T>(Cin, C, true);
+    if (nblocks < 1) return (int)hipErrorUnknown;
     HdP p;
     p.x = x; p.ps = pro_scale; p.pt = pro_shift; p.pslope = pro_scale ? (pro_slope < 0.f ? 1.f : pro_slope) : 1.f;
-    p.wp_fwd = wpf; p.wp_bwd = wpb; p.bias = bias; p.labels = labels; p.label_bytes = label_bytes;
+    p.w_io = w_io; p.bias = bias; p.labels = labels; p.label_bytes = label_bytes;
     p.V = V; p.N = N; p.K = Cin; p.C = C; p.partial = nullptr; p.coef = coef; p.dloss = dloss; p.dx = dx; p.wpartial = wpartial;
     const bool want_bst = bst && pro_scale && pro_mean && Cin == 16 && bst_cap >= nblocks && !DaEl<T>::bf;
     p.pmean = want_bst ? pro_mean : nullptr; p.bst = want_bst ? bst : nullptr;
-    if (want_bst && bst_n) *bst_n = nblocks;
+    const long long nchunks = da_cdiv(V, kHdChunk) * N;
+    if (want_bst && bst_n) *bst_n = (int)(nchunks < nblocks ? nchunks : nblocks);
     int rc;
     if (Cin == 16 && C == 32) rc = hd_launch_bwd<1, 2, T>(p, nblocks, st);
     else if (Cin == 16 && C == 16) rc = hd_launch_bwd<1, 1, T>(p, nblocks, st);
     else if (Cin == 64 && C == 32) rc = hd_launch_bwd<4, 2, T>(p, nblocks, st);
     else rc = hd_launch_bwd<4, 1, T>(p, nblocks, st);
     if (rc) return rc;
-    rc = da_reduce_partials(wpartial, nblocks, O, folded, st);
-    if (rc) return rc;
-    hipError_t e = hipMemcpyAsync(dw_io, folded, (size_t)Cin * C * sizeof(float), hipMemcpyDeviceToDevice, st);
-    if (e != hipSuccess) return (int)e;
-    if (dbias) { e = hipMemcpyAsync(dbias, folded + (size_t)Cin * C, (size_t)C * sizeof(float), hipMemcpyDeviceToDevice, st); if (e != hipSuccess) return (int)e; }
+    hipLaunchKernelGGL(hd_reduce_kernel, dim3((O + 15) / 16), dim3(256), 0, st, wpartial, nblocks, Cin * C, O, dw_io, dbias);
+    DA_LAUNCH_CHECK();
     return 0;
 }
 extern "C" int da_head_dice_bwd(const float* x, const float* pro_scale, const float* pro_shift, float pro_slope,
@@ -517,3 +573,9 @@
                                      int N, long long V, int Cin, int C, void* ws, size_t ws_bytes, void* stream) {
     return head_dice_bwd_t<da_bf16>((const float*)x, pro_scale, pro_shift, pro_slope, w_io, bias, labels, label_bytes, coef, dloss, (float*)dx, dw_io, dbias, N, V, Cin, C, ws, ws_bytes, stream);
 }
+
+extern "C" int da_head_dice_grid(int Cin, int C, int bf16, int bwd, int* chunk_voxels) {
+    if (!hd_shape_ok(Cin, C)) return 0;
+    if (chunk_voxels) *chunk_voxels = kHdChunk;
+    return bf16 ? hd_grid<da_bf16>(Cin, C, bwd != 0) : hd_grid<float>(Cin, C, bwd != 0);
+}
diff --git a/deepatlas_amd/csrc/losses.hip b/deepatlas_amd/csrc/losses.hip
--- a/deepatlas_amd/csrc/losses.hip
+++ b/deepatlas_amd/csrc/losses.hip
@@ -133,6 +133,7 @@
 __global__ void dice_finalize_kernel(const double* __restrict__ partial, int nblocks, int nsum, int N, int C,
                                      int weight_type, int no_bg, float eps, float* __restrict__ loss,
                                      float* __restrict__ coef, float* __restrict__ isc ) {
+    __shared__ float sh[2];
     const int NC = N * C;
     for (int i = threadIdx.x; i < 3 * NC; i += blockDim.x) {
         const int k = i / NC, nc = i % NC, n = nc / C, c = nc % C;
@@ -141,43 +142,59 @@
         isc[i] = (float)s;
     }
     __syncthreads();
-    if (threadIdx.x != 0) return;
     const float* I = isc; const float* S = isc + NC; const float* T = isc + 2 * NC;
     const int c0 = no_bg ? 1 : 0;
-    float wmax = -INFINITY;
-    for (int n = 0; n < N; ++n) {
-        float rowmax = -INFINITY;
-        for (int c = c0; c < C; ++c) {
-            float w;
-            if (weight_type == 1) w = 1.f / (powf(T[n * C + c], (float)(1.0 / 3.0)) + eps);
-            else if (weight_type == 2) w = 1.f / (T[n * C + c] + eps);
-            else w = 1.f;
-            coef[n * C + c] = w;
-            if (weight_type == 2) { const float t = isinf(w) ? 1.f : w; rowmax = fmaxf(rowmax, t); }
-        }
-        for (int c = c0; c < C; ++c) {
-            float w = coef[n * C + c];
-            if (weight_type == 2 && isinf(w)) { w = rowmax; coef[n * C + c] = w; }
-            wmax = fmaxf(wmax, w);
-        }
-    }
-    float wsum = 0.f, acc = 0.f;
-    for (int n = 0; n < N; ++n)
-        for (int c = c0; c < C; ++c) {
-            const float w = coef[n * C + c] / wmax;
-            coef[n * C + c] = w;
-            const float score = (2.f * I[n * C + c] + eps) / ((S[n * C + c] + T[n * C + c]) + 2.f * eps);
-            acc += w * score; wsum += w;
-        }
-    loss[0] = 1.f - acc / wsum;
-    for (int n = 0; n < N; ++n)
-        for (int c = 0; c < C; ++c) {
-            if (c < c0) { coef[n * C + c] = 0.f; coef[NC + n * C + c] = 0.f; continue; }
-            const float w = coef[n * C + c] / wsum;
-            const float den = (S[n * C + c] + T[n * C + c]) + 2.f * eps;
-            coef[n * C + c] = -w * 2.f / den;
-            coef[NC + n * C + c] = w * (2.f * I[n * C + c] + eps) / (den * den);
-        }
+    for (int nc = threadIdx.x; nc < NC; nc += blockDim.x) {
+        if (nc % C < c0) continue;
+        float w;
+        if (weight_type == 1) w = 1.f / (powf(T[nc], (float)(1.0 / 3.0)) + eps);
+        else if (weight_type == 2) w = 1.f / (T[nc] + eps);
+        else w = 1.f;
+        coef[nc] = w;
+    }
+    __syncthreads();
+    if (threadIdx.x == 0) {
+        float wmax = -INFINITY;
+        for (int n = 0; n < N; ++n) {
+            float rowmax = -INFINITY;
+            if (weight_type == 2)
+                for (int c = c0; c < C; ++c) { const float w = coef[n * C + c]; const float t = isinf(w) ? 1.f : w; rowmax = fmaxf(rowmax, t); }
+            for (int c = c0; c < C; ++c) {
+                float w = coef[n * C + c];
+                if (weight_type == 2 && isinf(w)) { w = rowmax; coef[n * C + c] = w; }
+                wmax = fmaxf(wmax, w);
+            }
+        }
+        sh[0] = wmax;
+    }
+    __syncthreads();
+    const float wmax = sh[0];
+    for (int nc = threadIdx.x; nc < NC; nc += blockDim.x) {
+        if (nc % C < c0) continue;
+        coef[nc] = coef[nc] / wmax;
+        coef[NC + nc] = (2.f * I[nc] + eps) / ((S[nc] + T[nc]) + 2.f * eps);
+    }
+    __syncthreads();
+    if (threadIdx.x == 0) {
+        float wsum = 0.f, acc = 0.f;
+        for (int n = 0; n < N; ++n)
+            for (int c = c0; c < C; ++c) {
+                const float w = coef[n * C + c];
+                const float score = coef[NC + n * C + c];
+                acc += w * score; wsum += w;
+            }
+        loss[0] = 1.f - acc / wsum;
+        sh[1] = wsum;
+    }
+    __syncthreads();
+    const float wsum = sh[1];
+    for (int nc = threadIdx.x; nc < NC; nc += blockDim.x) {
+        if (nc % C < c0) { coef[nc] = 0.f; coef[NC + nc] = 0.f; continue; }
+        const float w = coef[nc] / wsum;
+        const float den = (S[nc] + T[nc]) + 2.f * eps;
+        coef[nc] = -w * 2.f / den;
+        coef[NC + nc] = w * (2.f * I[nc] + eps) / (den * den);
+    }
 }
 
 __global__ void dice_bwd_vec_kernel(const float* __restrict__ src, const void* __restrict__ labels, int label_bytes,
diff --git a/include/deepatlas_hip.h b/include/deepatlas_hip.h
--- a/include/deepatlas_hip.h
+++ b/include/deepatlas_hip.h
@@ -211,6 +211,7 @@
                          const float* w_io, const float* bias, const void* labels, int label_bytes,
                          const float* coef, const float* dloss, float* dx, float* dw_io, float* dbias,
                          int N, long long V, int Cin, int C, double* bst, int bst_cap, int* bst_n, void* ws, size_t ws_bytes, void* stream);
+int da_head_dice_grid(int Cin, int C, int bf16, int bwd, int* chunk_voxels);
 
 int da_conv3d_k3_dgrad_bst(const float* dy, const float* w_tio, float* dx1, int C1, float* dx2, int C2, int N, int D, int H, int W, int Cout,
                            const float* y, const float* stats4, float slope, double* bst, int bst_cap, int* bst_n,
```
